# techpro-studio/NNToolkitCore

Hardware: AMD Instinct MI355X
Metric: audio frames/sec (whole node) (higher is better)
Workload: dtype f32

## Files before the change

include/nntoolkitcore_hip.h:

```cpp
#ifndef NNTOOLKITCORE_HIP_H
#define NNTOOLKITCORE_HIP_H

#include <stdbool.h>
#include <stddef.h>

#ifdef __cplusplus
extern "C" {
#endif


typedef struct { int mini_batch_size; } DefaultTrainingConfig;
typedef struct { int w; int b; int sum; } DefaultWeightsSize;
typedef struct { float *W; float *b; } DefaultWeights;

typedef void (*ActivationFunctionImpl)(void *, const float *, float *, int);
typedef void (*ActivationFunctionDerivative)(void *, const float *, const float *, float *, int);
typedef void (*ActivationImplementerDestroy)(void *);
typedef struct ActivationFunctionStruct *ActivationFunction;

ActivationFunction ActivationFunctionCreate(int size, ActivationImplementerDestroy destroy_fn, void *implementer,
                                            ActivationFunctionImpl function, ActivationFunctionDerivative derivative,
                                            ActivationFunctionDerivative cached_derivative);
void ActivationFunctionDestroy(ActivationFunction filter);
void ActivationFunctionApply(ActivationFunction filter, const float *input, float *output);
// ... 220 lines not shown
typedef struct {
    int nfft;
    int window_size;
    int noverlap;
    int step;
    int input_size;
    int nfreq;
    int ntime_series;
    float fft_normalization_factor;
} SpectrogramConfig;
typedef struct SpectrogramStruct *Spectrogram;

SpectrogramConfig SpectrogramConfigCreate(int nfft, int window_size, int noverlap, int input_size,
                                          float fft_normalization_factor);
Spectrogram SpectrogramCreatePSD(SpectrogramConfig config, int fs);
Spectrogram SpectrogramCreateMagnitude(SpectrogramConfig config);
SpectrogramConfig SpectrogramGetConfig(Spectrogram filter);
void SpectrogramSetWindowFunc(Spectrogram filter, window_fn fn);
void SpectrogramSetScaleFactor(Spectrogram filter, float factor);
void SpectrogramApply(Spectrogram filter, const float *input, float *output);
void SpectrogramDestroy(Spectrogram filter);

typedef struct {
    int n_mels;
    int n_fft;
    int sample_rate;
    float lower_hz;
    float upper_hz;
} MelFilterBankConfig;
typedef struct MelFilterBankStruct *MelFilterBank;
typedef struct LogMelSpectrogramStruct *LogMelSpectrogram;

MelFilterBankConfig MelFilterBankConfigCreate(int n_mels, int n_fft, int sample_rate, float lower_hz, float upper_hz);
MelFilterBank MelFilterBankCreate(MelFilterBankConfig config);
void MelFilterBankApply(MelFilterBank filter_bank, const float *spectrogram, float *mel_spectrogram, int timesteps);
void MelFilterBankDestroy(MelFilterBank filter_bank);
LogMelSpectrogram LogMelSpectrogramCreate(Spectrogram spectrogram, MelFilterBankConfig mel_filter_bank_config);
void LogMelSpectrogramApply(LogMelSpectrogram filter, const float *input, float *output);
void LogMelSpectrogramDestroy(LogMelSpectrogram filter);


int         nntk_hip_device_count(void);
int         nntk_hip_set_device(int device);
void        nntk_hip_set_stream(void *hip_stream);
void       *nntk_hip_get_stream(void);
int         nntk_hip_synchronize(void);
const char *nntk_last_error(void);
const char *nntk_version(void);
const char *nntk_build_source_hash(void);
int         nntk_hip_set_option(const char *name, const char *value);
int         nntk_hip_get_option(const char *name, int *value);
int         nntk_hip_device_status(void);
const char *nntk_hip_last_recurrent_kernel(void);
const char *nntk_hip_last_conv_kernel(void);
void        nntk_hip_profile_enable(int on);
int         nntk_hip_profile_get(const char *name, double *total_ms, long *launches, long *timesteps);

float *nntk_device_alloc(size_t n_floats);
void   nntk_device_free(float *ptr);
int    nntk_device_upload(float *dst_device, const float *src_host, size_t n_floats);
int    nntk_device_download(float *dst_host, const float *src_device, size_t n_floats);

int Conv1dSyncWeights(Conv1d filter);
int BatchNormSyncWeights(BatchNorm filter);
int GRUSyncWeights(GRU filter);
int LSTMSyncWeights(LSTM filter);
int RNNSyncWeights(RNN filter);
int DenseSyncWeights(Dense filter);
int TimeDistributedDenseSyncWeights(TimeDistributedDense filter);
int Conv1dLoadWeightsDevice(Conv1d filter, const float *d_block);
int BatchNormLoadWeightsDevice(BatchNorm filter, const float *d_block);
int GRULoadWeightsDevice(GRU filter, const float *d_block);
int LSTMLoadWeightsDevice(LSTM filter, const float *d_block);
int RNNLoadWeightsDevice(RNN filter, const float *d_block);
int DenseLoadWeightsDevice(Dense filter, const float *d_block);
int TimeDistributedDenseLoadWeightsDevice(TimeDistributedDense filter, const float *d_block);

#define NNTK_DIST_ID_BYTES 128
int  nntk_dist_get_unique_id(unsigned char id[NNTK_DIST_ID_BYTES]);
int  nntk_dist_init(const unsigned char id[NNTK_DIST_ID_BYTES], int rank, int world_size);
int  nntk_dist_rank(void);
int  nntk_dist_world_size(void);
int  nntk_dist_broadcast(float *host_block, size_t n_floats, int root);
int  nntk_dist_barrier(void);
int  nntk_dist_allreduce(float *host_block, size_t n_floats);
int  nntk_dist_allreduce_device(float *d_block, size_t n_floats);
int  nntk_dist_finalize(void);
void nntk_dist_shard_range(int n_utterances, int world_size, int rank, int *lo, int *hi);
int Conv1dBroadcastWeights(Conv1d filter, int root);
int BatchNormBroadcastWeights(BatchNorm filter, int root);
int GRUBroadcastWeights(GRU filter, int root);
int LSTMBroadcastWeights(LSTM filter, int root);
int RNNBroadcastWeights(RNN filter, int root);
int DenseBroadcastWeights(Dense filter, int root);
int TimeDistributedDenseBroadcastWeights(TimeDistributedDense filter, int root);

int Conv1dApplyInferenceBatch(Conv1d filter, const float *input, float *output, int batch);
int GRUApplyInferenceBatch(GRU filter, const float *input, float *output, int batch);
int LSTMApplyInferenceBatch(LSTM filter, const float *input, float *output, int batch);
int RNNApplyInferenceBatch(RNN filter, const float *input, float *output, int batch);
int TimeDistributedDenseApplyInferenceBatch(TimeDistributedDense filter, const float *input, float *output, int batch);
int SpectrogramApplyBatch(Spectrogram filter, const float *input, float *output, int batch);
int LogMelSpectrogramApplyBatch(LogMelSpectrogram filter, const float *input, float *output, int batch);

int SpectrogramApplyDevice(Spectrogram filter, const float *d_input ,
                           float *d_output , int batch);
// ... 267 lines not shown
```

nntoolkitcore_amd/capi.py:

```python
import ctypes as C
import os

_PKG = os.path.dirname(os.path.abspath(__file__))
LIB_PATH = os.path.join(_PKG, "lib", "libnntoolkitcore_hip.so")
if os.environ.get("NNTK_LIB"):
    LIB_PATH = os.path.abspath(os.environ["NNTK_LIB"])

fp = C.POINTER(C.c_float)
vp = C.c_void_p


class Conv1dConfig(C.Structure):
    _fields_ = [("input_feature_channels", C.c_int), ("output_feature_channels", C.c_int),
                ("kernel_size", C.c_int), ("stride", C.c_int), ("input_size", C.c_int), ("output_size", C.c_int)]


class ConvTrainingConfig(C.Structure):
    _fields_ = [("mini_batch_size", C.c_int)]


class DefaultGradient(C.Structure):
    _fields_ = [("d_W", fp), ("d_b", fp), ("d_X", fp)]


# ... 203 lines not shown
    "DenseGradientDestroy": (None, [C.POINTER(DefaultGradient)]),
    "DenseCalculateGradient": (None, [vp, C.POINTER(DefaultGradient), fp]),
    "ActivationFunctionCalculateGradient": (None, [vp, fp, fp, fp, fp]),
    "ActivationFunctionCalculateGradientDevice": (C.c_int, [vp, vp, vp, vp, vp, C.c_int]),
    "mean_squared_error": (C.c_float, [fp, fp, C.c_int, C.c_int]),
    "mean_squared_error_derivative": (None, [fp, fp, fp, C.c_int, C.c_int]),
    "categorical_crossentropy": (C.c_float, [fp, fp, C.c_int, C.c_int]),
    "categorical_crossentropy_derivative": (None, [fp, fp, fp, C.c_int, C.c_int]),
    "sgd_optimize": (C.c_int, [SGD, fp, fp, C.c_int]),
    "nntk_mean_squared_error_device": (C.c_int, [vp, vp, C.c_int, C.c_int, C.POINTER(C.c_float)]),
    "nntk_categorical_crossentropy_device": (C.c_int, [vp, vp, C.c_int, C.c_int, C.POINTER(C.c_float)]),
    "nntk_mean_squared_error_derivative_device": (C.c_int, [vp, vp, vp, C.c_int, C.c_int]),
    "nntk_categorical_crossentropy_derivative_device": (C.c_int, [vp, vp, vp, C.c_int, C.c_int]),
    "nntk_sgd_optimize_device": (C.c_int, [SGD, vp, vp, C.c_long]),
    "DenseDestroy": (None, [vp]),
    "TimeDistributedDenseConfigCreate": (TimeDistributedDenseConfig, [C.c_int, DenseConfig]),
    "TimeDistributedDenseCreateForInference": (vp, [TimeDistributedDenseConfig]),
    "TimeDistributedDenseGetWeights": (C.POINTER(DefaultWeights), [vp]),
    "TimeDistributedDenseApplyInference": (C.c_int, [vp, fp, fp]),
    "TimeDistributedDenseDestroy": (None, [vp]),
    "hamming_window": (None, [fp, C.c_int]),
    "hann_window": (None, [fp, C.c_int]),
    "ones": (None, [fp, C.c_int]),
    "periodic_hamming_window": (None, [fp, C.c_int]),
    "periodic_hann_window": (None, [fp, C.c_int]),
    "blackman_window": (None, [fp, C.c_int]),
    "SpectrogramConfigCreate": (SpectrogramConfig, [C.c_int, C.c_int, C.c_int, C.c_int, C.c_float]),
    "SpectrogramCreatePSD": (vp, [SpectrogramConfig, C.c_int]),
    "SpectrogramCreateMagnitude": (vp, [SpectrogramConfig]),
    "SpectrogramGetConfig": (SpectrogramConfig, [vp]),
    "SpectrogramSetWindowFunc": (None, [vp, vp]),
    "SpectrogramSetScaleFactor": (None, [vp, C.c_float]),
    "SpectrogramApply": (None, [vp, fp, fp]),
    "SpectrogramDestroy": (None, [vp]),
    "MelFilterBankConfigCreate": (MelFilterBankConfig, [C.c_int, C.c_int, C.c_int, C.c_float, C.c_float]),
    "MelFilterBankCreate": (vp, [MelFilterBankConfig]),
    "MelFilterBankApply": (None, [vp, fp, fp, C.c_int]),
    "MelFilterBankDestroy": (None, [vp]),
    "LogMelSpectrogramCreate": (vp, [vp, MelFilterBankConfig]),
    "LogMelSpectrogramApply": (None, [vp, fp, fp]),
    "LogMelSpectrogramDestroy": (None, [vp]),
    "nntk_hip_device_count": (C.c_int, []),
    "nntk_hip_set_device": (C.c_int, [C.c_int]),
    "nntk_hip_set_stream": (None, [vp]),
    "nntk_hip_get_stream": (vp, []),
    "nntk_hip_synchronize": (C.c_int, []),
    "nntk_last_error": (C.c_char_p, []),
    "nntk_version": (C.c_char_p, []),
    "nntk_build_source_hash": (C.c_char_p, []),
    "nntk_hip_set_option": (C.c_int, [C.c_char_p, C.c_char_p]),
    "nntk_hip_get_option": (C.c_int, [C.c_char_p, C.POINTER(C.c_int)]),
    "nntk_hip_device_status": (C.c_int, []),
    "nntk_hip_last_recurrent_kernel": (C.c_char_p, []),
    "nntk_hip_last_conv_kernel": (C.c_char_p, []),
    "nntk_hip_profile_enable": (None, [C.c_int]),
    "nntk_hip_profile_get": (C.c_int, [C.c_char_p, C.POINTER(C.c_double), C.POINTER(C.c_long), C.POINTER(C.c_long)]),
    "nntk_device_alloc": (vp, [C.c_size_t]),
    "nntk_device_free": (None, [vp]),
    "nntk_device_upload": (C.c_int, [vp, fp, C.c_size_t]),
    "nntk_device_download": (C.c_int, [fp, vp, C.c_size_t]),
    "nntk_dist_get_unique_id": (C.c_int, [C.c_char_p]),
    "nntk_dist_init": (C.c_int, [C.c_char_p, C.c_int, C.c_int]),
    "nntk_dist_rank": (C.c_int, []),
    "nntk_dist_world_size": (C.c_int, []),
    "nntk_dist_broadcast": (C.c_int, [fp, C.c_size_t, C.c_int]),
    "nntk_dist_barrier": (C.c_int, []),
    "nntk_dist_allreduce": (C.c_int, [fp, C.c_size_t]),
    "nntk_dist_allreduce_device": (C.c_int, [vp, C.c_size_t]),
    "nntk_dist_finalize": (C.c_int, []),
    "nntk_dist_shard_range": (None, [C.c_int, C.c_int, C.c_int, C.POINTER(C.c_int), C.POINTER(C.c_int)]),
    "Conv1dBroadcastWeights": (C.c_int, [vp, C.c_int]),
    "BatchNormBroadcastWeights": (C.c_int, [vp, C.c_int]),
    "GRUBroadcastWeights": (C.c_int, [vp, C.c_int]),
    "LSTMBroadcastWeights": (C.c_int, [vp, C.c_int]),
    "RNNBroadcastWeights": (C.c_int, [vp, C.c_int]),
    "DenseBroadcastWeights": (C.c_int, [vp, C.c_int]),
    "TimeDistributedDenseBroadcastWeights": (C.c_int, [vp, C.c_int]),
    "Conv1dSyncWeights": (C.c_int, [vp]),
    "BatchNormSyncWeights": (C.c_int, [vp]),
    "GRUSyncWeights": (C.c_int, [vp]),
    "LSTMSyncWeights": (C.c_int, [vp]),
    "RNNSyncWeights": (C.c_int, [vp]),
    "DenseSyncWeights": (C.c_int, [vp]),
    "TimeDistributedDenseSyncWeights": (C.c_int, [vp]),
    "Conv1dApplyInferenceBatch": (C.c_int, [vp, fp, fp, C.c_int]),
    "GRUApplyInferenceBatch": (C.c_int, [vp, fp, fp, C.c_int]),
    "LSTMApplyInferenceBatch": (C.c_int, [vp, fp, fp, C.c_int]),
    "RNNApplyInferenceBatch": (C.c_int, [vp, fp, fp, C.c_int]),
    "TimeDistributedDenseApplyInferenceBatch": (C.c_int, [vp, fp, fp, C.c_int]),
    "SpectrogramApplyBatch": (C.c_int, [vp, fp, fp, C.c_int]),
    "LogMelSpectrogramApplyBatch": (C.c_int, [vp, fp, fp, C.c_int]),
    "MelFilterBankApplyDevice": (C.c_int, [vp, vp, vp, C.c_int]),
    "LogMelSpectrogramApplyDevice": (C.c_int, [vp, vp, vp, C.c_int]),
    "SpectrogramApplyDevice": (C.c_int, [vp, vp, vp, C.c_int]),
    "Conv1dApplyDevice": (C.c_int, [vp, vp, vp, C.c_int]),
    "Conv1dBatchNormActivationApplyDevice": (C.c_int, [vp, vp, vp, vp, vp, C.c_int]),
    "Conv1dBatchNormActivationApplyDeviceFrag3": (C.c_int, [vp, vp, vp, vp, vp, C.c_int]),
    "BatchNormApplyDevice": (C.c_int, [vp, vp, vp, C.c_int]),
    "ActivationFunctionApplyDevice": (C.c_int, [vp, vp, vp, C.c_int]),
    "GRUApplyDevice": (C.c_int, [vp, vp, vp, C.c_int]),
    "GRUStack2ApplyDevice": (C.c_int, [vp, vp, vp, vp, C.c_int]),
    "GRUStack2ApplyInferenceBatch": (C.c_int, [vp, vp, fp, fp, C.c_int]),
    "LSTMApplyDevice": (C.c_int, [vp, vp, vp, C.c_int]),
    "nntk_frag3_floats": (C.c_size_t, [C.c_int, C.c_int, C.c_int]),
    "nntk_frag3_pack_device": (C.c_int, [vp, vp, C.c_int, C.c_int, C.c_int]),
    "nntk_frag3_unpack_device": (C.c_int, [vp, vp, C.c_int, C.c_int, C.c_int]),
# ... 194 lines not shown
```

nntoolkitcore_amd/csrc/hip/nntk_common.hpp:

```cpp
#pragma once
#include <hip/hip_runtime.h>
#include <math.h>
#include "nntk_shim.h"

hipStream_t nntk_stream();
int nntk_fail(const char *what, hipError_t err);
int nntk_fail_msg(const char *what);
enum { NNTK_SPAN_REC = 0, NNTK_SPAN_SPEC = 1 };
int nntk_prof_span_begin(int kind);
void nntk_prof_span_end(int idx, long launches, long units);

struct NntkOptions {
    int rec_persistent = -1;
    int rec_xw = -1;
    int rec_pingpong = -1;
    int rec_groups = 2;
    int rec_spin_us = 1000000;
    int rec_stream = -1;
    int rec_fused2 = -1;
    int rec_rr = -1;
    int rec_xf = -1;
    int rec_fk = -1;
    int rec_hf = -1;
    int rec_hf_pend = 1;
    int rec_bd = -1;
    int dense_frag3 = -1;
    int dense_f16x2 = -1;
    int train_outer_plain = -1;
    int train_bptt = -1;
    int spec_ppw = 0;
    int spec_variant = -1;
#ifdef NNTK_VARIANT_SPEC_DMA
    int spec_dma = -1;
#endif
    int bn_fast = 0;
    int gemm_tm_batch = -1;
    int conv_a4 = 1;
    int conv_flatk = -1;
    int conv_frag3_out = -1;
    int conv_store = -1;
    int gemm_split_bf16 = -1;
    int gemm_wide = -1;
    int conv_dbg = 0;
    int weights_check = -1;
};
const NntkOptions &nntk_options();

unsigned *nntk_fault_word();
int nntk_fault_enqueue_copy();
int nntk_persistent_disabled();
void nntk_persistent_launch_begin();
void nntk_persistent_launch_end();
bool nntk_weights_exact_only(const void *d_wp);
int nntk_cu_count();
void nntk_set_last_conv_kernel(const char *name);
void nntk_set_last_rec_kernel(const char *name);
int nntk_set_max_dynamic_lds(const void *kernel, size_t bytes);
int nntk_outer_mfma_launch(const float *d_A, const float *d_B, float *d_partial, long rows, int I, int K, int a_shift_T,
                           long rps, long seq_pitch, long row_pitch);
int nntk_resident_blocks(const void *kernel, int threads, size_t lds, int max_per_cu);

#define NNTK_STR_(x) #x
#define NNTK_STR(x) NNTK_STR_(x)

#define NNTK_HIP_TRY(expr)                                             \
    do {                                                               \
        hipError_t _e = (expr);                                        \
        if (_e != hipSuccess) return nntk_fail(#expr, _e);             \
    } while (0)

#define NNTK_LAUNCH_CHECK(name)                                        \
    do {                                                               \
        hipError_t _e = hipGetLastError();                             \
        if (_e != hipSuccess) return nntk_fail(name, _e);              \
    } while (0)

typedef float f32x4 __attribute__((ext_vector_type(4)));
typedef float f32x16 __attribute__((ext_vector_type(16)));

__device__ __forceinline__ float nntk_act(int kind, float x, float relu_a) {
    switch (kind) {
    case NNTK_ACT_SIGMOID: return 1.0f / (1.0f + expf(-x));
    case NNTK_ACT_TANH:    return tanhf(x);
    case NNTK_ACT_RELU: {
        float y = fmaxf(x, 0.0f);
        return relu_a != 1.0f ? y * relu_a : y;
    }
    case NNTK_ACT_LOG_EPS: return logf(x + relu_a);
    default: return x;
    }
}

__device__ __forceinline__ float nntk_fast_sigmoid(float x) {
    return __builtin_amdgcn_rcpf(1.0f + __builtin_amdgcn_exp2f(-1.44269504088896341f * x));
}
__device__ __forceinline__ float nntk_fast_tanh(float x) {
    const float e = __builtin_amdgcn_exp2f(-2.88539008177792681f * fabsf(x));
    const float r = (1.0f - e) * __builtin_amdgcn_rcpf(1.0f + e);
    return copysignf(r, x);
}
__device__ __forceinline__ float nntk_gate_act(int kind, float x, float a = 1.0f) {
    switch (kind) {
    case NNTK_ACT_SIGMOID: return nntk_fast_sigmoid(x);
    case NNTK_ACT_TANH:    return nntk_fast_tanh(x);
    case NNTK_ACT_RELU: {
        const float y = fmaxf(x, 0.0f);
        return a != 1.0f ? y * a : y;
    }
    default: return x;
// ... 5 lines not shown
```

nntoolkitcore_amd/csrc/hip/nntk_shim.h:

```cpp
#ifndef NNTK_SHIM_H
#define NNTK_SHIM_H

#include <stddef.h>

#ifdef __cplusplus
extern "C" {
#endif

enum {
    NNTK_ACT_NONE     = -1,
    NNTK_ACT_IDENTITY = 0,
    NNTK_ACT_SIGMOID  = 1,
    NNTK_ACT_TANH     = 2,
    NNTK_ACT_RELU     = 3,
    NNTK_ACT_SOFTMAX  = 4,
    NNTK_ACT_LOG_EPS  = 5,
    NNTK_ACT_CUSTOM   = 100
};

int         nntk_shim_device_count(void);
int         nntk_shim_set_device(int device);
int         nntk_shim_get_device(void);
void        nntk_shim_set_stream(void *stream);
void       *nntk_shim_get_stream(void);
int         nntk_shim_synchronize(void);
const char *nntk_shim_error(void);
void        nntk_shim_set_error(const char *msg);
void        nntk_shim_clear_error(void);

int nntk_shim_set_option(const char *name, const char *value);
int nntk_shim_get_option(const char *name, int *value);
int nntk_shim_take_fault(void);
int nntk_shim_persistent_disabled(void);
const char *nntk_shim_last_conv_kernel(void);
const char *nntk_shim_last_rec_kernel(void);
int nntk_shim_device_status(void);

void nntk_shim_profile_enable(int on);
int  nntk_shim_profile_get(const char *name, double *total_ms, long *launches, long *timesteps);

void *nntk_shim_malloc(size_t bytes);
void  nntk_shim_free(void *d_ptr);
void *nntk_shim_host_alloc(size_t bytes);
void  nntk_shim_host_free(void *ptr);
int   nntk_shim_upload(void *d_dst, const void *h_src, size_t bytes);
int   nntk_shim_upload_async(void *d_dst, const void *h_src, size_t bytes);
int   nntk_shim_download(void *h_dst, const void *d_src, size_t bytes);
int   nntk_shim_download_nocheck(void *h_dst, const void *d_src, size_t bytes);
int   nntk_shim_download_rows(void *h_dst, const void *d_src, size_t spitch, size_t width, size_t height);
int   nntk_shim_copy_d2d(void *d_dst, const void *d_src, size_t bytes);
int   nntk_shim_copy_rows_d2d(void *d_dst, const void *d_src, size_t spitch, size_t width, size_t height);
int   nntk_shim_memset(void *d_ptr, int value, size_t bytes);

void nntk_shim_conv_pack_sizes(int Cin, int Cout, int k, int *Cin_p, int *Cout_p);
int  nntk_shim_bn_derive(float *d_block, float eps, int C);
int  nntk_shim_split_bf16x3(const float *d_src, void *d_dst, int rows, int ktot);
void nntk_shim_weights_exact_only(const void *d_wp, int on);
int  nntk_shim_conv1d(const float *d_in, const float *d_wp, const float *d_bias, const float *d_bn,
                      float bn_eps, int act_kind, float relu_a, float *d_out,
                      int B, int T, int Cin, int Cout, int k, int stride, int Tout, int out_mode);

int  nntk_shim_conv1d_frag3(const float *d_in, const float *d_wp, const float *d_bias, const float *d_bn,
                            float bn_eps, int act_kind, float relu_a, float *d_out_f3,
                            int B, int T, int Cin, int Cout, int k, int stride, int Tout);
int nntk_shim_conv1d_flatk(const float *d_in, const float *d_wpf, const float *d_bias, const float *d_bn,
                           float bn_eps, int act_kind, float relu_a, float *d_out,
                           int B, int T, int Cin, int Cout, int k, int Tout);
size_t nntk_shim_conv1d_grad_scratch_floats(int Cin, int Cout, int k);
int nntk_shim_conv1d_grad(const float *d_in, const float *d_W, const float *d_dout, float *d_dW, float *d_db,
                          float *d_dX, float *d_scratch, int B, int T, int Cin, int Cout, int k, int stride, int Tout);

int nntk_shim_batch_norm(const float *d_in, const float *d_bn , float eps,
                         float *d_out, long rows, int C);
int nntk_shim_activation(int kind, float relu_a, int softmax_vector_size,
                         const float *d_in, float *d_out, long n_elems);

int nntk_shim_reverse_time(const float *d_in, float *d_out, long B, int T, int F);
int nntk_shim_reverse_time_varlen(const float *d_in, float *d_out, const int *d_len, long B, int T, int F);
int nntk_shim_upload_ints(int *d_dst, const int *h_src, long n);
int nntk_shim_stream_gather(const float *d_in, float *d_state, float *d_seq, const int *d_cnt, int B, int in_rows, int state_rows, int C);
int nntk_shim_spectrogram_rows(const float *d_in, const float *d_window, const float *d_twiddle, float *d_out,
                               int B, int row_stride, int nfft, int window_size, int step, int nfreq, int max_frames,
                               float fft_norm, int mode, float scale, const int *d_cnt,
                               const int *d_mel_tab, const float *d_mel_w, int n_mels, float eps, int do_log);
int nntk_shim_activation_grad(int kind, int vector_size, int vectors_per_call, const float *d_z, const float *d_a,
                              const float *d_dout, float *d_out, long n);
int nntk_shim_dense_grad(const float *d_x, const float *d_W , const float *d_dz, float *d_gW,
// ... 118 lines not shown
int nntk_shim_split2(const float *d_in, float *d_a, float *d_b, long rows, int C);
int nntk_shim_bd_merge(const float *d_of, const float *d_obr, float *d_out, const int *d_len, long B, int T, int H,
                       int return_sequences, int concat);
int nntk_shim_bd_scatter(const float *d_dout, float *d_of, float *d_ob, const int *d_len, long B, int T, int H,
                         int return_sequences, int concat, int reverse);
int nntk_shim_bd_accumulate(const float *d_dxf, const float *d_dxbr, float *d_dx, const int *d_len, long B, int T, int F);

int nntk_shim_rnn(const float *d_xw, const float *d_ut, const float *d_bh, const float *d_h0,
                  float *d_out, float *d_hT, float *d_work, int B, int T, int H,
                  int return_sequences, int act, float act_scale);
size_t nntk_shim_recurrent_work_floats(int B, int H);
int nntk_shim_rec_varlen(int G, const float *d_xw, const float *d_ut, const float *d_bh, const float *d_h0,
                         const float *d_c0, float *d_out, float *d_hT, float *d_cT, float *d_work, int B, int T, int H,
                         int return_sequences, const int *acts, const float *act_scales, const int *d_len, int T_max);
int nntk_shim_varlen_zero_pad(float *d_out, const int *d_len, int B, int T, int H);
int nntk_shim_gru(const float *d_xw, const float *d_ut, const float *d_bh,
                  const float *d_h0, float *d_out, float *d_hT, float *d_work,
                  int B, int T, int H, int return_sequences, const int acts[3], const float act_scales[3]);
int nntk_shim_lstm(const float *d_xw, const float *d_ut, const float *d_bh,
                   const float *d_h0, const float *d_c0, float *d_out, float *d_hT, float *d_cT,
                   float *d_work, int B, int T, int H, int return_sequences, const int acts[5], const float act_scales[5]);

size_t nntk_shim_lstm_rr_image_floats(int H, int in);
size_t nntk_shim_rr_image_floats_xf(int H, int in);
size_t nntk_shim_lstm_rr_work_floats(int B, int H);
size_t nntk_shim_rr_hseq_floats(int B, int T, int H);
int nntk_shim_lstm_rr_pack(const float *d_ut, const float *d_wp, float *d_img, int H, int in);
int nntk_shim_lstm_rr_pack_raw(const float *d_U , const float *d_W , float *d_img, int H, int in);
size_t nntk_shim_fk_image_floats(int H, int in);
int nntk_shim_fk_pack(const float *d_ut, const float *d_wp, float *d_img4, int H, int in);
int nntk_shim_fk_pack_raw(const float *d_U , const float *d_W , float *d_img4, int H, int in);
int nntk_shim_gru_rr(const float *d_x, const void *d_xf3, const float *d_img, const float *d_img4, const float *d_b4, const float *d_h0, float *d_out,
                     float *d_hseq, float *d_hT, float *d_work, int B, int T, int in, int H, int return_sequences, int x_tm, int out_tm);
int nntk_shim_gru_rr_train_forward(const float *d_x, const float *d_img, const float *d_b4, float *d_h, float *d_hU, float *d_Zg,
                                   float *d_hseq, float *d_work, int B, int T, int in, int H);
int nntk_shim_lstm_rr_train_forward(const float *d_x, const float *d_img, const float *d_bi, const float *d_bh,
                                    float *d_h, float *d_c, float *d_zifgo, float *d_hseq, float *d_work, int B, int T, int in, int H);
int nntk_shim_lstm_rr(const float *d_x, const void *d_xf3, const float *d_img, const float *d_img4, const float *d_bi, const float *d_bh,
                      const float *d_h0, const float *d_c0, float *d_out, float *d_out_h2 ,
                      float *d_hseq, float *d_hT, float *d_cT, float *d_work, int B, int T, int in, int H, int return_sequences);

int nntk_shim_rr_varlen(int cell, const float *d_x, const void *d_xf3, const float *d_img, const float *d_img4, const float *d_bi,
                        const float *d_bh, const float *d_h0, const float *d_c0, float *d_out, float *d_hseq, float *d_hT, float *d_cT,
                        float *d_work, const int *d_len, int B, int T, int in, int H, int return_sequences);

int nntk_shim_rr_bd(int cell, const void *d_xf3, const float *d_img, const float *d_img4, const float *d_bi, const float *d_bh,
                    const float *d_img_b, const float *d_img4_b, const float *d_bi_b, const float *d_bh_b, float *d_out, float *d_out_b,
                    int ldo, float *d_hseq, float *d_work, const int *d_len, int B, int T, int in, int H, int return_sequences);
int nntk_shim_rr_bd_fits(int T, int in, int ldo);

int nntk_shim_lstm_rr_hf_ok(int H, int in);
size_t nntk_shim_lstm_rr_hf_image_floats(int H, int in);
int nntk_shim_lstm_rr_pack_hf(const float *d_ut, const float *d_wp, float *d_img, int H, int in, float uscale, float wscale);
int nntk_shim_lstm_rr_hf(const void *d_xf3, const float *d_img, const float *d_bi, const float *d_bh, float *d_h2, float *d_work,
                         int B, int T, int in, int H, float z_scale);

size_t nntk_shim_frag3_floats(int B, int T, int C);
int nntk_shim_frag3_pack(const float *d_x, void *d_frag, int B, int T, int C);
int nntk_shim_frag3_pack_bd(const float *d_x, const int *d_len, void *d_frag, int B, int T, int C);
int nntk_shim_frag3_unpack(const void *d_frag, float *d_x, int B, int T, int C);
size_t nntk_shim_frag2h_floats(int B, int T, int C);
int nntk_shim_frag2h_pack(const float *d_x, void *d_frag, int B, int T, int C);
int nntk_shim_frag2h_unpack(const void *d_frag, float *d_x, int B, int T, int C);
int nntk_shim_split_f16x2(const float *d_src, void *d_dst, int rows, int ktot, float scale);
int nntk_shim_dense_frag2h(const void *d_frag, const void *d_wh2, float w_scale, const float *d_bias, int act_kind, float relu_a,
                           float *d_out, int B, int T, int K, int N, int probe);
int nntk_shim_dense_frag3(const void *d_frag, const float *d_wp, const float *d_bias, int act_kind, float relu_a,
                          float *d_out, int B, int T, int K, int N);

size_t nntk_shim_gru2_work_floats(int B, int H);
int nntk_shim_gru2(const float *d_xw1, const float *d_ut1, const float *d_bh1, const float *d_wt2,
                   const float *d_bi2, const float *d_ut2, const float *d_bh2, float *d_out, float *d_out1,
                   float *d_work, int B, int T, int H, int return_sequences);

int nntk_shim_rec_stream(int G, int is_lstm, const float *x, const float *d_wp, const float *d_bi,
                         const float *d_ut, const float *d_bh, float *d_h0, float *d_h1, float *d_c0, float *d_c1,
                         int cur, float *out, int T, int in, int H, int return_sequences,
                         const int *acts, const float *scales, unsigned *d_done, unsigned *flag, unsigned seq);

int nntk_shim_dist_unique_id(unsigned char *id128);
int nntk_shim_dist_init(const unsigned char *id128, int rank, int world);
int nntk_shim_dist_rank(void);
int nntk_shim_dist_world(void);
int nntk_shim_dist_broadcast_host(float *block, size_t n, int root);
int nntk_shim_add_into(float *d_dst, const float *d_src, long n);
int nntk_shim_dist_barrier(void);
int nntk_shim_dist_allreduce_device(float *d_block, size_t n);
int nntk_shim_dist_allreduce_host(float *block, size_t n);
int nntk_shim_dist_finalize(void);

int nntk_shim_spectrogram(const float *d_in, const float *d_window, const float *d_twiddle, float *d_out,
                          int B, int input_size, int nfft, int window_size, int step,
                          int nfreq, int nts, float fft_norm, int mode, float scale);

int nntk_shim_spectrogram_mel(const float *d_in, const float *d_window, const float *d_twiddle, float *d_out,
                              int B, int input_size, int nfft, int window_size, int step,
                              int nfreq, int nts, float fft_norm, int mode, float scale,
                              const int *d_mel_tab, const float *d_mel_w, int n_mels, float eps, int do_log);

#ifdef __cplusplus
}
#endif
#endif
```

nntoolkitcore_amd/csrc/hip/recurrent_fk.hip:

```cpp
#include "recurrent_rr_common.hpp"

typedef unsigned fk_v2u __attribute__((ext_vector_type(2)));
template <int LO, int HI, class F>
__device__ __forceinline__ void fk_for(F &&f) {
    if constexpr (LO < HI) {
        f(std::integral_constant<int, LO>{});
        fk_for<LO + 1, HI>(f);
    }
}
__host__ __device__ constexpr int fk_ring(int NKX, int NW) { return NW == 4 && NKX > 8 ? 2 : 4; }
#ifndef FK_ND_4
#define FK_ND_4 3
#endif
#ifndef FK_ND_4W
#define FK_ND_4W 4
#endif
#ifndef FK_LEAD_CAP
#define FK_LEAD_CAP 0
#endif
#ifndef FK_FIN_SLICED
#define FK_FIN_SLICED 0
#endif
#ifndef FK_FIN_VALU
#define FK_FIN_VALU 5
#endif
#ifndef FK_ND_2
#define FK_ND_2 8
#endif

#ifdef NNTK_REC_STAMPS
#ifndef FK_FINE_GS
#define FK_FINE_GS 2
#endif
#define FK_FINE(gs, k) do { if ((gs) == FK_FINE_GS) asm volatile("s_memtime %0" : "=s"(fine[k])); } while (0)
#define FK_FINE_OUT(gs, t) do { if ((gs) == FK_FINE_GS) { asm volatile("s_waitcnt lgkmcnt(0)" ::: "memory"); \
        if (p.stamp && blockIdx.x == 0 && w == 0 && lane == 0 && (t) >= 0) { for (int k_ = 0; k_ < 10; ++k_) p.stamp[(size_t)(t) * 64 + 48 + k_] = fine[k_]; } } } while (0)
#define FK_STAMP(t, i) do { if (p.stamp && blockIdx.x == 0 && w == 0 && lane == 0 && (t) >= 0) \
        p.stamp[(size_t)(t) * 64 + (i)] = __builtin_amdgcn_s_memtime(); } while (0)
#else
#define FK_STAMP(t, i) do {} while (0)
#define FK_FINE(gs, k) do {} while (0)
#define FK_FINE_OUT(gs, t) do {} while (0)
#endif

__host__ __device__ inline int fk_blocks_per_ct(int NKH, int NKX, int NW) { return NW * (NKH * 3 + NKX * 3); }
__host__ __device__ inline int fk_nmr(int NKH) { return NKH <= 16 ? 3 : 2; }
__host__ __device__ inline int fk_nmw(int NKX, int NW) { return NW == 4 && NKX > 8 ? 1 : 0; }
__host__ __device__ inline int fk_walk(int NGP, int NW, int ct, int ug, int pos) {
    const int g = pos / NW, j = pos % NW;
    return NW * ((g + ct) % NGP) + ((ug ^ j ^ (ct / NGP)) & (NW - 1));
}

template <bool RAW>
__global__ __launch_bounds__(256) void fk_pack_kernel(const float *__restrict__ ut, const float *__restrict__ wp,
                                                      rr_v4u *__restrict__ img, int H, int in, int Hj_p, int Hk_p, int Kin_p,
                                                      int NKH, int NKX, int NMR, int NW, int NCT) {
    const int NMW = fk_nmw(NKX, NW);
    const int n_ur = NW * NKH * NMR, n_wr = NW * NKX * NMW, n_ul = NW * NKH * (3 - NMR), bpc = fk_blocks_per_ct(NKH, NKX, NW);
    const long total = (long)NCT * bpc * 64;
    for (long e = blockIdx.x * (long)blockDim.x + threadIdx.x; e < total; e += (long)gridDim.x * blockDim.x) {
        const int l = (int)(e & 63);
        const long blk = e >> 6;
        const int ct = (int)(blk / bpc);
        int r = (int)(blk % bpc);
        int part, ug, pos, m;
        if (r < n_ur) { part = 0; m = r % NMR; pos = (r / NMR) % NKH; ug = r / (NMR * NKH); }
        else if (r < n_ur + n_wr) { r -= n_ur; part = 2; m = r % NMW; pos = (r / NMW) % NKX; ug = r / (NMW * NKX); }
        else if (r < n_ur + n_wr + n_ul) { r -= n_ur + n_wr; part = 0; const int nl = 3 - NMR; m = NMR + r % nl; pos = (r / nl) % NKH; ug = r / (nl * NKH); }
        else { r -= n_ur + n_wr + n_ul; part = 2; const int nl = 3 - NMW; m = NMW + r % nl; pos = (r / nl) % NKX; ug = r / (nl * NKX); }
        const int ks = fk_walk(part == 2 ? NKX / NW : NKH / NW, NW, ct, ug, pos);
        const int c = l & 31;
        const int g = c >> 3;
        const int j = 8 * (NW * ct + ug) + (c & 7);
        float v[8];
#pragma unroll
        for (int q = 0; q < 8; ++q) {
            const int k = 16 * ks + 8 * (l >> 5) + q;
            float val = 0.0f;
            if (j < H) {
                if (RAW) {
                    if (part == 2) { if (k < in) val = wp[(size_t)k * 4 * H + (size_t)g * H + j]; }
                    else if (k < H) val = ut[(size_t)k * 4 * H + (size_t)g * H + j];
                } else {
                    if (part == 2) { if (k < in) val = wp[((size_t)g * H + j) * Kin_p + k]; }
                    else if (k < H) val = ut[((size_t)g * Hj_p + j) * Hk_p + k];
                }
            }
            v[q] = val;
        }
        rr_v4u hi, mid, lo;
        rr_split8(v, hi, mid, lo);
        img[e] = m == 0 ? hi : m == 1 ? mid : lo;
    }
}

template <int NKH, int NKX, int CELL, int NW, int ND, bool VL = false, bool BD = false>
__device__ __forceinline__ void fk_body(const RRParams &p) {
    static_assert(!BD || VL, "BD: per-row lengths");
    constexpr int NMR = NKH <= 16 ? 3 : 2;
    constexpr int NMW = NW == 4 && NKX > 8 ? 1 : 0;
    constexpr int FK_RING = fk_ring(NKX, NW);
    constexpr bool BURST = FK_RING == 2;
    constexpr int NGH = NKH / NW, NGX = NKX / NW, NG = NGH + NGX;
    constexpr int NHF = 4 / NW;
    static_assert((NW == 2 || NW == 4) && NKH % NW == 0 && NKX % NW == 0 && NGX >= 1, "group schedule");
    static_assert((2 * NG) % ND == 0 && (2 * NG) % fk_ring(NKX, NW) == 0 && ND <= NGH, "staging / ring indices repeat every two steps at most");
    constexpr auto fk_lead = [](int q) constexpr {
        if (q >= NGH) return ND;
        if (!FK_LEAD_CAP) return ND;
        const int want = 2 + (q + 1) / 2, cap = NGX + q;
        const int l = want < cap ? want : cap;
        return l < ND ? l : ND;
    };
    constexpr int FIN_G = NW == 4 ? 1 : (NGX >= 4 ? 4 : NGX);
    extern __shared__ __attribute__((aligned(16))) char smem[];
    rr_v4u *ULs = reinterpret_cast<rr_v4u *>(smem);
    rr_v4u *WXs = ULs + NW * NKH * (3 - NMR) * 64;
    rr_v4u *ring = WXs + NW * NKX * (3 - NMW) * 64;
    unsigned *flg = reinterpret_cast<unsigned *>(ring + 4 * FK_RING * 3 * 64);
#define FK_FENCE() asm volatile("" ::: "memory")

    const int tid = threadIdx.x;
    const int lane = tid & 63;
    const int w = __builtin_amdgcn_readfirstlane(tid >> 6);
    const int hf = w / NW, ug = w % NW;
    const int n = lane & 31, kh = lane >> 5;
    const int bt = blockIdx.x % p.NBT;
    const int ct = blockIdx.x / p.NBT;
    const int ht_abs = p.b_base / 32 + bt * NHF + hf;
    const int b0 = p.b_base + bt * 32 * NHF;
    const int H = p.H;
    const int T = VL ? __builtin_amdgcn_readfirstlane(p.len[p.B + (b0 >> 6)]) : p.T;
    const int NKS = H >> 4;
    const bool bwd = BD && b0 >= p.bd_pad;
    const int rb0 = bwd ? b0 - p.bd_pad : b0;
    const int rows_valid = BD ? (p.bd_rows - rb0 < 32 * NHF ? (p.bd_rows > rb0 ? p.bd_rows - rb0 : 0) : 32 * NHF)
                              : p.B - b0 < 32 * NHF ? p.B - b0 : 32 * NHF;
    const int gi = NW * ct + ug;
    if (VL && T == 0) {
        if constexpr (BD) rr_bd_pass_state(p, b0, 32 * NHF, 8 * NW * ct, 8 * NW);
        else rr_vl_pass_state(p, b0, 32 * NHF, 8 * NW * ct, 8 * NW, CELL == 0);
        return;
    }
    const bool grp_ok = 8 * gi < H;

    const rr_v4u *img = (bwd ? p.img_b : p.img) + (size_t)ct * fk_blocks_per_ct(NKH, NKX, NW) * 64;
    rr_bf16x8 uh[NKH][NMR];
#pragma unroll
    for (int pos = 0; pos < NKH; ++pos)
#pragma unroll
        for (int m = 0; m < NMR; ++m) {
            uh[pos][m] = __builtin_bit_cast(rr_bf16x8, img[(((size_t)ug * NKH + pos) * NMR + m) * 64 + lane]);
            RR_PIN_A(uh[pos][m]);
        }
    rr_bf16x8 wr[NMW ? NKX : 1][NMW ? NMW : 1];
    if (NMW) {
#pragma unroll
        for (int pos = 0; pos < NKX; ++pos)
#pragma unroll
            for (int m = 0; m < NMW; ++m) {
                wr[pos][m] = __builtin_bit_cast(rr_bf16x8, img[(size_t)NW * NKH * NMR * 64 + (((size_t)ug * NKX + pos) * NMW + m) * 64 + lane]);
            }
    }
    {
        const rr_v4u *src = img + (size_t)(NW * NKH * NMR + NW * NKX * NMW) * 64;
        constexpr int n16 = (NW * NKH * (3 - NMR) + NW * NKX * (3 - NMW)) * 64;
        for (int e = tid; e < n16; e += 256) ULs[e] = src[e];
        for (int e = tid; e < 4 * FK_RING * 64; e += 256) flg[e] = 0u;
    }
    const int jf = 8 * gi + 4 * kh;
    float bsum[4][4];
    const float *const bi = bwd ? p.bi_b : p.bi, *const bh = bwd ? p.bh_b : p.bh;
#pragma unroll
    for (int g = 0; g < 4; ++g)
#pragma unroll
        for (int e = 0; e < 4; ++e)
            bsum[g][e] = jf + e < H ? bi[g * H + jf + e] + (bh ? bh[g * H + jf + e] : 0.0f) : 0.0f;
    float cst[4];
    {
        const int row = b0 + hf * 32 + n;
#pragma unroll
        for (int e = 0; e < 4; ++e) cst[e] = (p.c0 && row < p.B && jf + e < H) ? p.c0[(size_t)row * H + jf + e] : 0.0f;
    }
    int vlen = 0;
    float hkeep[VL && CELL == 0 ? 4 : 1];
    if constexpr (VL) {
        const int row = b0 + hf * 32 + n;
        vlen = row < p.B ? p.len[row] : 0;
        if constexpr (CELL == 0) {
#pragma unroll
            for (int e = 0; e < 4; ++e) hkeep[e] = (p.h0 && row < p.B && jf + e < H) ? p.h0[(size_t)row * H + jf + e] : 0.0f;
        }
    }
    const int hb_bytes = (int)p.hstep;
    auto rs_rd = [&](int t) __attribute__((always_inline)) {
        return __builtin_amdgcn_make_buffer_rsrc((void *)(t ? p.hseq + (size_t)(t - 1) * p.hstep : p.h0f), 0, t < T ? hb_bytes : 0, 0x00020000);
    };
    auto rs_wr = [&](int t) __attribute__((always_inline)) {
        return __builtin_amdgcn_make_buffer_rsrc((void *)(p.hseq + (size_t)t * p.hstep), 0, hb_bytes, 0x00020000);
    };
    auto rs_x = [&](int t) __attribute__((always_inline)) {
#ifdef FK_X_HOT
        return __builtin_amdgcn_make_buffer_rsrc((void *)(p.xf3), 0, t < T ? (int)p.xstep : 0, 0x00020000);
#endif
        return __builtin_amdgcn_make_buffer_rsrc((void *)(p.xf3 + (size_t)(t < T ? t : 0) * p.xstep), 0, t < T ? (int)p.xstep : 0, 0x00020000);
    };
    const int lane16 = lane * 16;
    const int ugh = (ug ^ (ct / NGH)) & (NW - 1), ugx = (ug ^ (ct / NGX)) & (NW - 1);
    const int hso = ht_abs * NKS * 3 * 1024;
    const int xso = ht_abs * p.NKSx * 3 * 1024;
    const int ldo = BD ? p.ldo : H;
    const long o_row_bytes = (long)(p.return_sequences ? p.T : 1) * ldo * 4;
    const long o_range = rows_valid * o_row_bytes;
    const __amdgpu_buffer_rsrc_t rso = __builtin_amdgcn_make_buffer_rsrc(
        (void *)((bwd ? p.out_b : p.out) + (size_t)rb0 * (o_row_bytes / 4)), 0, (int)(o_range < 0x7fffffffL ? o_range : 0x7fffffffL), 0x00020000);
    const bool row_ok = hf * 32 + n < rows_valid && grp_ok;
    const int out_vo = row_ok ? (int)((hf * 32 + n) * o_row_bytes) + jf * 4 : 0x7fff0000;
    const int pub_vo = grp_ok ? ((ht_abs * NKS + (gi >> 1)) * 3) * 1024 + (32 * (gi & 1) + n) * 16 + 8 * kh : RR_OOB_F;
    RR_BARRIER();

    using Tt = std::true_type;
    using Ff = std::false_type;
    using I0 = std::integral_constant<int, 0>;
    using I1 = std::integral_constant<int, 1>;
    rr_v4u S[ND][3];
    rr_v4u P[NW - 1][3];
    unsigned fl[NW - 1];
    rr_bf16x8 wa[2][3];
    rr_bf16x8 ulo[2];

    auto issue_own = [&](int g_h, int g_x, bool is_h, int si, int tq, int m0 = 0, int m1 = 3) __attribute__((always_inline)) {
        if (RR_DBG(1)) return;
        if (is_h) {
            const __amdgpu_buffer_rsrc_t rs = rs_rd(tq);
            const int ks = NW * ((g_h + ct) % NGH) + ugh;
            const int so = hso + ks * 3072;
            const int vo = lane16 + (ks < NKS ? 0 : RR_OOB_F);
#pragma unroll
            for (int m = 0; m < 3; ++m) {
                if (m < m0 || m >= m1) continue;
                S[si][m] = __builtin_amdgcn_raw_buffer_load_b128(rs, vo + m * 1024, so, 16 );
                RR_BOUND(tq ? 3 : 4, tq ? (size_t)(tq - 1) * p.hstep : 0, vo + m * 1024, so, tq < T ? hb_bytes : 0, 16);
            }
        } else {
            const __amdgpu_buffer_rsrc_t rs = rs_x(tq + 1);
            const int ks = NW * ((g_x + ct) % NGX) + ugx;
            const int so = xso + ks * 3072;
            const int vo = lane16 + (ks < p.NKSx ? 0 : RR_OOB_F);
#pragma unroll
            for (int m = 0; m < 3; ++m) {
                if (m < m0 || m >= m1) continue;
                S[si][m] = __builtin_amdgcn_raw_buffer_load_b128(rs, vo + m * 1024, so, 0);
                RR_BOUND(1, (size_t)(tq + 1) * p.xstep, vo + m * 1024, so, tq + 1 < T ? p.xstep : 0, 16);
            }
        }
    };
    auto probe = [&](int si) __attribute__((always_inline)) {
        unsigned mx = 0;
#pragma unroll
        for (int m = 0; m < 3; ++m) {
            const rr_v4u v = S[si][m];
            mx = max(mx, max(max(v.x, v.y), max(v.z, v.w)));
        }
        return __builtin_amdgcn_ballot_w64(mx == RR_PENDING);
    };
    const unsigned long long inject = p.spin_ticks == 0 ? ~0ull : 0ull;
    auto settle = [&](int g_h, int si, int tq) __attribute__((always_inline)) {
        {
            const unsigned long long t_start = __builtin_amdgcn_s_memrealtime();
            bool expired = p.spin_ticks == 0;
            while (!expired) {
                issue_own(g_h, 0, true, si, tq);
                if (probe(si) == 0) break;
                if (__hip_atomic_load(p.fault, __ATOMIC_RELAXED, __HIP_MEMORY_SCOPE_AGENT) != 0) { expired = true; break; }
                __builtin_amdgcn_s_sleep(1);
                expired = __builtin_amdgcn_s_memrealtime() - t_start > p.spin_ticks;
            }
            if (expired && lane == 0) __hip_atomic_fetch_or(p.fault, 1u, __ATOMIC_RELAXED, __HIP_MEMORY_SCOPE_AGENT);
        }
    };
    auto ring_put = [&](int si, int slot, unsigned seq, int piece) __attribute__((always_inline)) {
        rr_v4u *d = ring + ((w * FK_RING + slot) * 3) * 64 + lane;
        FK_FENCE();
#pragma unroll
        for (int m = 0; m < 3; ++m)
            if (piece < 0 || piece == m) d[m * 64] = S[si][m];
        FK_FENCE();
        if (piece < 0 || piece == 2) flg[(w * FK_RING + slot) * 64 + lane] = seq;
        FK_FENCE();
    };
    auto ring_word = [&](int j, int slot) __attribute__((always_inline)) {
        const int pw = hf * NW + (ug ^ j);
        FK_FENCE();
        fl[j - 1] = flg[(pw * FK_RING + slot) * 64 + lane];
        FK_FENCE();
    };
    auto ring_data = [&](int j, int slot, int m0, int m1) __attribute__((always_inline)) {
        const int pw = hf * NW + (ug ^ j);
        const rr_v4u *s = ring + ((pw * FK_RING + slot) * 3) * 64 + lane;
        FK_FENCE();
#pragma unroll
        for (int m = 0; m < 3; ++m)
            if (m >= m0 && m < m1) P[j - 1][m] = s[m * 64];
        FK_FENCE();
    };
    auto ring_check = [&](int slot, unsigned seq) __attribute__((always_inline)) {
        bool bad = false;
#pragma unroll
        for (int j = 1; j < NW; ++j) bad |= fl[j - 1] != seq;
        if (__builtin_amdgcn_ballot_w64(bad) != 0) {
            const unsigned long long t_start = __builtin_amdgcn_s_memrealtime();
            bool expired = false;
            while (!expired) {
                bad = false;
#pragma unroll
                for (int j = 1; j < NW; ++j) { ring_word(j, slot); bad |= fl[j - 1] != seq; }
                if (__builtin_amdgcn_ballot_w64(bad) == 0) break;
                if (__hip_atomic_load(p.fault, __ATOMIC_RELAXED, __HIP_MEMORY_SCOPE_AGENT) != 0) { expired = true; break; }
                __builtin_amdgcn_s_sleep(1);
                expired = __builtin_amdgcn_s_memrealtime() - t_start > p.spin_ticks;
            }
            if (expired && lane == 0) __hip_atomic_fetch_or(p.fault, 1u, __ATOMIC_RELAXED, __HIP_MEMORY_SCOPE_AGENT);
#pragma unroll
            for (int j = 1; j < (BURST ? NW : 2); ++j) ring_data(j, slot, 0, 3);
        }
    };
    float hn[4];
    rr_v4u olast = {0u, 0u, 0u, 0u};
    auto fin_unit = [&](int e, const f32x16 &acc, int t) __attribute__((always_inline)) {
        if (RR_DBG(2)) return;
        float zc[4];
#pragma unroll
        for (int g = 0; g < 4; ++g) zc[g] = acc[4 * g + e] + bsum[g][e];
        if (RR_DBG(64)) { hn[e] = zc[0] + zc[1] + zc[2] + zc[3] + cst[e]; return; }
        if (CELL == 1) {
            const float zg = nntk_fast_sigmoid(zc[0]);
            const float rg = nntk_fast_sigmoid(zc[1]);
            const float ht = nntk_fast_tanh(fmaf(rg, zc[2], zc[3]));
            hn[e] = fmaf(-zg + 1.0f, ht, zg * cst[e]);
            if constexpr (VL) hn[e] = t < vlen ? hn[e] : cst[e];
            cst[e] = hn[e];
        } else {
            const float ig = nntk_fast_sigmoid(zc[0]);
            const float fg = nntk_fast_sigmoid(zc[1]);
            const float gg = nntk_fast_tanh(zc[2]);
            const float og = nntk_fast_sigmoid(zc[3]);
            const float cn = fmaf(fg, cst[e], ig * gg);
            if constexpr (VL) {
                const bool live = t < vlen;
                hn[e] = live ? og * nntk_fast_tanh(cn) : hkeep[e];
                cst[e] = live ? cn : cst[e];
                hkeep[e] = hn[e];
            } else {
            cst[e] = cn;
            hn[e] = og * nntk_fast_tanh(cn);
            }
        }
    };
    auto fin_store = [&](int t) __attribute__((always_inline)) {
        if (RR_DBG(2)) return;
        if (!RR_DBG(128)) {
            unsigned sh0, sm0, sl0, sh1, sm1, sl1;
            rr_split_pair(hn[0], hn[1], sh0, sm0, sl0);
            rr_split_pair(hn[2], hn[3], sh1, sm1, sl1);
            const fk_v2u a = {(unsigned)min(sh0, 0xfffffffeu), (unsigned)min(sh1, 0xfffffffeu)};
            const fk_v2u b = {(unsigned)min(sm0, 0xfffffffeu), (unsigned)min(sm1, 0xfffffffeu)};
            const fk_v2u c = {(unsigned)min(sl0, 0xfffffffeu), (unsigned)min(sl1, 0xfffffffeu)};
            const __amdgpu_buffer_rsrc_t rs = rs_wr(t);
            __builtin_amdgcn_raw_buffer_store_b64(a, rs, pub_vo, 0, RR_ST_AUX );
            __builtin_amdgcn_raw_buffer_store_b64(b, rs, pub_vo + 1024, 0, RR_ST_AUX);
            __builtin_amdgcn_raw_buffer_store_b64(c, rs, pub_vo + 2048, 0, RR_ST_AUX);
            RR_BOUND(3, (size_t)t * p.hstep, pub_vo + 2048, 0, hb_bytes, 8);
        }
        olast = (rr_v4u){__float_as_uint(hn[0]), __float_as_uint(hn[1]), __float_as_uint(hn[2]), __float_as_uint(hn[3])};
        if (!RR_DBG(1024)) {
            int vo = (row_ok && p.return_sequences && p.out) ? out_vo + t * H * 4 : 0x7fff0000;
            if constexpr (BD)
                vo = (row_ok && p.return_sequences && t < vlen) ? out_vo + (bwd ? vlen - 1 - t : t) * ldo * 4 : 0x7fff0000;
            __builtin_amdgcn_raw_buffer_store_b128(olast, rso, vo, 0, 0);
            RR_BOUND(2, (size_t)b0 * o_row_bytes, vo, 0, o_range < 0x7fffffffL ? o_range : 0x7fffffffL, 16);
        }
    };

    auto mark_next = [&](int t) __attribute__((always_inline)) {
        if (RR_DBG(128)) return;
        const __amdgpu_buffer_rsrc_t rs2 = rs_wr(t + 1 < T ? t + 1 : t);
        const int vo2 = t + 1 < T ? pub_vo : RR_OOB_F;
        const fk_v2u pend = {RR_PENDING, RR_PENDING};
        __builtin_amdgcn_raw_buffer_store_b64(pend, rs2, vo2, 0, RR_ST_AUX);
        __builtin_amdgcn_raw_buffer_store_b64(pend, rs2, vo2 + 1024, 0, RR_ST_AUX);
        __builtin_amdgcn_raw_buffer_store_b64(pend, rs2, vo2 + 2048, 0, RR_ST_AUX);
        RR_BOUND(3, (size_t)(t + 1 < T ? t + 1 : t) * p.hstep, vo2 + 2048, 0, hb_bytes, 8);
    };

    constexpr int PA[6] = {0, 2, 1, 0, 1, 0}, PB[6] = {2, 0, 1, 1, 0, 0};
    auto lds_fetch_a = [&](bool is_h, int pos, int buf) __attribute__((always_inline)) {
        if (is_h) {
            if (NMR == 2) ulo[buf] = __builtin_bit_cast(rr_bf16x8, ULs[(ug * NKH + pos) * 64 + lane]);
        } else {
#pragma unroll
            for (int m = NMW; m < 3; ++m) wa[buf][m] = __builtin_bit_cast(rr_bf16x8, WXs[((ug * NKX + pos) * (3 - NMW) + (m - NMW)) * 64 + lane]);
        }
    };
    auto mult = [&](f32x16 &acc, bool is_h, int pos, int buf, const rr_v4u (&bsrc)[3], int j0, int j1) __attribute__((always_inline)) {
        if (RR_DBG(16)) return;
        rr_bf16x8 b[3];
#pragma unroll
        for (int m = 0; m < 3; ++m) b[m] = __builtin_bit_cast(rr_bf16x8, bsrc[m]);
#pragma unroll
        for (int pr = 0; pr < 6; ++pr) {
            if (pr < j0 || pr >= j1) continue;
            rr_bf16x8 av;
            if (is_h) av = (NMR == 2 && PA[pr] == 2) ? ulo[buf] : uh[pos][PA[pr] < NMR ? PA[pr] : 0];
            else av = PA[pr] < NMW ? wr[NMW ? pos : 0][NMW ? PA[pr] : 0] : wa[buf][PA[pr]];
            acc = __builtin_amdgcn_mfma_f32_32x32x16_bf16(av, b[PB[pr]], acc, 0, 0, 0);
        }
    };

    auto issue_sched = [&](int gs, int par, int t, int k, int m0, int m1) __attribute__((always_inline)) {
        int seen = 0;
#pragma unroll
        for (int L = 1; L <= ND; ++L) {
            const int r = gs + L, q = r % NG;
            if (fk_lead(q) != L) continue;
            if (seen++ != k) continue;
            const bool qh = q < NGH;
            issue_own(qh ? q : 0, qh ? 0 : q - NGH, qh, (par * NG + r) % ND, t + r / NG, m0, m1);
        }
    };
    auto step = [&](auto par_tag, auto hp_tag, int t, f32x16 &acc, f32x16 &accn) __attribute__((always_inline)) {
        constexpr int PAR = decltype(par_tag)::value;
        constexpr bool HP = decltype(hp_tag)::value;
        fk_for<(HP ? 0 : NGH), NG>([&](auto gs_tag) __attribute__((always_inline)) {
            constexpr int gs = decltype(gs_tag)::value;
            const bool is_h = gs < NGH;
            const int pos0 = NW * (is_h ? gs : gs - NGH);
            const int gidx = PAR * NG + gs;
            const int si = gidx % ND, slot = gidx % FK_RING;
            const int si1 = (gidx + 1) % ND, slot1 = (gidx + 1) % FK_RING;
            const unsigned seq = (unsigned)((t + 1) * NG + gs) + 1u;
            const int q1 = (gs + 1) % NG, t1 = t + (gs + 1 >= NG ? 1 : 0);
            const bool h1 = q1 < NGH;
            f32x16 &a = is_h ? acc : accn;
            FK_STAMP(t, gs);
            if (gs == NGH) {
#pragma unroll
                for (int r = 0; r < 16; ++r) accn[r] = 0.0f;
            }
#define FK_PIN() __builtin_amdgcn_sched_barrier(0)
            const bool LATE = FK_LEAD_CAP && gs == NG - 1;
            const bool chk1 = h1 && !LATE && !RR_DBG(4) && !RR_DBG(1);
            unsigned mx0 = 0, mx1 = 0, mx2 = 0;
#ifdef NNTK_REC_STAMPS
            unsigned long long fine[10] = {0, 0, 0, 0, 0, 0, 0, 0, 0, 0};
#endif
            FK_FINE(gs, 0);
            mult(a, is_h, pos0, 0, S[si], 0, 1); FK_PIN();
#pragma unroll
            for (int j = 1; j < NW; ++j) ring_word(j, slot);
            if (chk1) { const rr_v4u v = S[si1][0]; mx0 = max(max(v.x, v.y), max(v.z, v.w)); asm volatile("" : "+v"(mx0)); }
            FK_PIN();
            mult(a, is_h, pos0, 0, S[si], 1, 2); FK_PIN();
            ring_data(1, slot, 0, 3);
            if (BURST && NW == 4) ring_data(2, slot, 0, 3);
            if (chk1) { const rr_v4u v = S[si1][1]; mx1 = max(mx0, max(max(v.x, v.y), max(v.z, v.w))); asm volatile("" : "+v"(mx1)); }
            FK_PIN();
            mult(a, is_h, pos0, 0, S[si], 2, 3); FK_PIN();
            if (BURST && NW == 4) ring_data(3, slot, 0, 3);
            if (chk1) { const rr_v4u v = S[si1][2]; mx2 = max(mx1, max(max(v.x, v.y), max(v.z, v.w))); asm volatile("" : "+v"(mx2)); }
            lds_fetch_a(is_h, pos0 + 1, 1); FK_PIN();
            FK_FINE(gs, 1);
            {
                bool bad = false;
                if (!RR_DBG(512)) {
#pragma unroll
                    for (int j = 1; j < NW; ++j) bad |= fl[j - 1] != seq;
                }
                unsigned long long pend = chk1 ? __builtin_amdgcn_ballot_w64(mx2 == RR_PENDING) | inject : 0ull;
                if (t1 <= 0) pend = 0ull;
                if (__builtin_expect((pend | __builtin_amdgcn_ballot_w64(bad)) != 0, 0)) {
                    if (pend != 0) settle(q1, si1, t1);
                    if (!RR_DBG(512)) ring_check(slot, seq);
                }
            }
            FK_FINE(gs, 2);
#ifdef FK_COARSE_GS
            if (gs == FK_COARSE_GS) FK_STAMP(t, 40);
#endif
            if (!RR_DBG(512) && !LATE) ring_put(si1, slot1, seq + 1u, 0);
            FK_PIN();
            mult(a, is_h, pos0, 0, S[si], 3, 4); FK_PIN();
            if (!RR_DBG(512) && !LATE) ring_put(si1, slot1, seq + 1u, 1);
            FK_PIN();
            mult(a, is_h, pos0, 0, S[si], 4, 5); FK_PIN();
            if (!RR_DBG(512) && !LATE) ring_put(si1, slot1, seq + 1u, 2);
            FK_PIN();
            mult(a, is_h, pos0, 0, S[si], 5, 6); FK_PIN();
            if (HP && gs == 0) { mark_next(t); FK_PIN(); }
#ifdef FK_COARSE_GS
            if (gs == FK_COARSE_GS) FK_STAMP(t, 41);
#endif
            FK_FINE(gs, 3);
            const int gx = gs - NGH;
            const bool fin_here = FK_FIN_SLICED && HP && !is_h && gx < FIN_G;
#pragma unroll
            for (int j = 1; j < NW; ++j) {
                mult(a, is_h, pos0 + j, j & 1, P[j - 1], 0, 2); if (!fin_here) FK_PIN();
                if (j + 1 < NW && !BURST) ring_data(j + 1, slot, 0, 1);
                issue_sched(gs, PAR, t, j - 1, 0, 1); if (!fin_here) FK_PIN();
                if (j + 1 < NW) lds_fetch_a(is_h, pos0 + j + 1, (j + 1) & 1);
                else lds_fetch_a(h1, NW * (h1 ? q1 : q1 - NGH), 0);
                if (!fin_here) FK_PIN();
                mult(a, is_h, pos0 + j, j & 1, P[j - 1], 2, 4); if (!fin_here) FK_PIN();
                if (j + 1 < NW && !BURST) ring_data(j + 1, slot, 1, 2);
                issue_sched(gs, PAR, t, j - 1, 1, 2); if (!fin_here) FK_PIN();
                mult(a, is_h, pos0 + j, j & 1, P[j - 1], 4, 6); if (!fin_here) FK_PIN();
                if (j + 1 < NW && !BURST) ring_data(j + 1, slot, 2, 3);
                issue_sched(gs, PAR, t, j - 1, 2, 3); if (!fin_here) FK_PIN();
                FK_FINE(gs, 3 + j);
#ifdef FK_COARSE_GS
                if (gs == FK_COARSE_GS) FK_STAMP(t, 41 + j);
#endif
            }
#pragma unroll
            for (int k = NW - 1; k < 3; ++k) issue_sched(gs, PAR, t, k, 0, 3);
            if (fin_here) {
#pragma unroll
                for (int e = 0; e < 4; ++e)
                    if (e * FIN_G / 4 == gx) fin_unit(e, acc, t);
                if (gx == FIN_G - 1) fin_store(t);
#pragma unroll
                for (int k = 0; k < 6 * (NW - 1); ++k) {
                    __builtin_amdgcn_sched_group_barrier(0x008, 1, 0);
                    __builtin_amdgcn_sched_group_barrier(0x002, FK_FIN_VALU, 0);
                    if (k % 2 == 1) __builtin_amdgcn_sched_group_barrier(0x030, 1, 0);
                    else __builtin_amdgcn_sched_group_barrier(0x100, 1, 0);
                }
            }
            if (LATE) {
                if (h1 && t1 > 0 && !RR_DBG(4) && !RR_DBG(1)) {
                    const unsigned long long pend = probe(si1) | inject;
                    if (__builtin_expect(pend != 0, 0)) settle(q1, si1, t1);
                }
                if (!RR_DBG(512)) ring_put(si1, slot1, seq + 1u, -1);
            }
            __builtin_amdgcn_sched_barrier(0);
            FK_FINE_OUT(gs, t);
            if (!FK_FIN_SLICED && HP && gs == NGH - 1) {
#pragma unroll
                for (int e = 0; e < 4; ++e) fin_unit(e, acc, t);
                fin_store(t);
                FK_STAMP(t, 33);
                __builtin_amdgcn_sched_barrier(0);
            }
            if (FK_FIN_SLICED && HP && !is_h && gx == FIN_G - 1) FK_STAMP(t, 33);
        });
    };

    f32x16 accA, accB;
#pragma unroll
    for (int r = 0; r < 16; ++r) { accA[r] = 0.0f; accB[r] = 0.0f; }
    {
#pragma unroll
        for (int r = NGH; r < NGH + ND; ++r) {
            const int q = r % NG;
            if (r - fk_lead(q) >= NGH) continue;
            const bool qh = q < NGH;
            issue_own(qh ? q : 0, qh ? 0 : q - NGH, qh, (NG + r) % ND, -1 + r / NG);
        }
        ring_put((NG + NGH) % ND, (NG + NGH) % FK_RING, (unsigned)NGH + 1u, -1);
        lds_fetch_a(false, 0, 0);
    }
    step(I1{}, Ff{}, -1, accB, accA);
    for (int t = 0; t < T; t += 2) {
        step(I0{}, Tt{}, t, accA, accB);
        if (t + 1 >= T) break;
        step(I1{}, Tt{}, t + 1, accB, accA);
    }
    if constexpr (BD) {
        int b0e = rb0;
        asm volatile("" : "+s"(b0e));
        const int row = b0e + hf * 32 + n;
        if (row < p.bd_rows && grp_ok && !p.return_sequences)
            *reinterpret_cast<rr_v4u *>((bwd ? p.out_b : p.out) + (size_t)row * ldo + jf) = olast;
    } else {
        int b0e = b0;
        asm volatile("" : "+s"(b0e));
        const int row = b0e + hf * 32 + n;
        if (row < p.B && grp_ok) {
            if (!p.return_sequences && p.out) *reinterpret_cast<rr_v4u *>(p.out + (size_t)row * H + jf) = olast;
            if (p.hT) *reinterpret_cast<rr_v4u *>(p.hT + (size_t)row * H + jf) = olast;
            if (p.cT) *reinterpret_cast<rr_v4u *>(p.cT + (size_t)row * H + jf) =
                (rr_v4u){__float_as_uint(cst[0]), __float_as_uint(cst[1]), __float_as_uint(cst[2]), __float_as_uint(cst[3])};
        }
    }
}
template <int NKH, int NKX, int NW, int ND, bool VL = false, bool BD = false>
__global__ __launch_bounds__(256) void lstm_fk_kernel(RRParams p) { fk_body<NKH, NKX, 0, NW, ND, VL, BD>(p); }
template <int NKH, int NKX, int NW, int ND, bool VL = false, bool BD = false>
__global__ __launch_bounds__(256) void gru_fk_kernel(RRParams p) { fk_body<NKH, NKX, 1, NW, ND, VL, BD>(p); }

static bool fk_shape(int H, int in, int *NKH, int *NKX, int *NW) {
    if ((H % 16) != 0 || H <= 128 || H > 256 || in <= 64 || in > 256) return false;
    const int on = nntk_options().rec_fk;
    if (on == 0 || (on < 0 && in <= 128)) return false;
    *NKH = 16;
    *NKX = in <= 128 ? 8 : 16;
    *NW = 4;
#ifdef FK_NW2_WIDE
    if (in > 128) *NW = 2;
#endif
    return true;
}
static size_t fk_lds_bytes(int NKH, int NKX, int NW) {
    return (size_t)(NW * NKH * (3 - fk_nmr(NKH)) + NW * NKX * (3 - fk_nmw(NKX, NW)) + 4 * fk_ring(NKX, NW) * 3) * 1024 + 4 * fk_ring(NKX, NW) * 64 * 4;
}
extern "C" size_t nntk_shim_fk_image_floats(int H, int in) {
    int NKH, NKX, NW;
    if (!fk_shape(H, in, &NKH, &NKX, &NW)) return 0;
    return (size_t)((H + 8 * NW - 1) / (8 * NW)) * fk_blocks_per_ct(NKH, NKX, NW) * 256;
}
static int fk_pack(bool raw, const float *d_u, const float *d_w, float *d_img, int H, int in) {
    int NKH, NKX, NW;
    if (!fk_shape(H, in, &NKH, &NKX, &NW)) return nntk_fail_msg("fk_pack: shape not taken by the full-K register-resident kernel");
    const int Hj_p = (H + 15) & ~15, Hk_p = (H + 31) & ~31;
    int Kin_p, N_p;
    nntk_shim_conv_pack_sizes(in, 4 * H, 1, &Kin_p, &N_p);
    const int NCT = (H + 8 * NW - 1) / (8 * NW), NMR = NKH <= 16 ? 3 : 2;
    const long total = (long)NCT * fk_blocks_per_ct(NKH, NKX, NW) * 64;
    long g = (total + 255) / 256;
    if (g > 4096) g = 4096;
    if (raw) hipLaunchKernelGGL(fk_pack_kernel<true>, dim3((unsigned)g), dim3(256), 0, nntk_stream(), d_u, d_w, (rr_v4u *)d_img, H, in, 0, 0, 0, NKH, NKX, NMR, NW, NCT);
    else     hipLaunchKernelGGL(fk_pack_kernel<false>, dim3((unsigned)g), dim3(256), 0, nntk_stream(), d_u, d_w, (rr_v4u *)d_img, H, in, Hj_p, Hk_p, Kin_p, NKH, NKX, NMR, NW, NCT);
    NNTK_LAUNCH_CHECK("fk_pack_kernel");
    return 0;
}
extern "C" int nntk_shim_fk_pack(const float *d_ut, const float *d_wp, float *d_img, int H, int in) { return fk_pack(false, d_ut, d_wp, d_img, H, in); }
extern "C" int nntk_shim_fk_pack_raw(const float *d_U, const float *d_W, float *d_img, int H, int in) { return fk_pack(true, d_U, d_W, d_img, H, in); }

int nntk_fk_launch(RRParams q, const float *d_imgfk, const float *d_imgfk_b, int cell, size_t *launches) {
    int NKH, NKX, NW;
    if (!d_imgfk || !q.xf3 || q.x_tm || q.out_tm || !fk_shape(q.H, q.in, &NKH, &NKX, &NW)) return 1;
    const bool bd = q.out_b != nullptr;
    if (bd && (!d_imgfk_b || !q.len)) return 1;
    void (*kern)(RRParams) = nullptr;
    if (bd) {
        if (cell == 1) kern = NKX == 8 ? gru_fk_kernel<16, 8, 4, FK_ND_4, true, true> : gru_fk_kernel<16, 16, 4, FK_ND_4W, true, true>;
        else kern = NKX == 8 ? lstm_fk_kernel<16, 8, 4, FK_ND_4, true, true> : lstm_fk_kernel<16, 16, 4, FK_ND_4W, true, true>;
    } else if (q.len) {
        if (cell == 1) kern = NKX == 8 ? gru_fk_kernel<16, 8, 4, FK_ND_4, true> : gru_fk_kernel<16, 16, 4, FK_ND_4W, true>;
        else kern = NKX == 8 ? lstm_fk_kernel<16, 8, 4, FK_ND_4, true> : lstm_fk_kernel<16, 16, 4, FK_ND_4W, true>;
    } else if (cell == 1) kern = NKX == 8 ? gru_fk_kernel<16, 8, 4, FK_ND_4> : gru_fk_kernel<16, 16, 4, FK_ND_4W>;
    else kern = NKX == 8 ? lstm_fk_kernel<16, 8, 4, FK_ND_4> : lstm_fk_kernel<16, 16, 4, FK_ND_4W>;
#ifdef FK_NW2_WIDE
    if (NW == 2 && (q.len || bd)) return 1;
    if (NW == 2) kern = cell == 1 ? gru_fk_kernel<16, 16, 2, FK_ND_2> : lstm_fk_kernel<16, 16, 2, FK_ND_2>;
#endif
    const size_t lds = fk_lds_bytes(NKH, NKX, NW);
    if (lds > 160 * 1024) return 1;
    if (nntk_set_max_dynamic_lds((const void *)kern, lds)) return -1;
    const int NCT = (q.H + 8 * NW - 1) / (8 * NW);
    const int rows = 128 / NW;
    const int resident = nntk_resident_blocks((const void *)kern, 256, lds, 1);
    const int tiles_per_launch = resident / NCT;
    if (tiles_per_launch < 1) return 1;
    q.img = (const rr_v4u *)d_imgfk;
    if (bd) q.img_b = (const rr_v4u *)d_imgfk_b;
    q.NCT = NCT;
    const int nbt_total = (q.B + rows - 1) / rows;
    for (int bt0 = 0; bt0 < nbt_total; bt0 += tiles_per_launch) {
        const int nbt = nbt_total - bt0 < tiles_per_launch ? nbt_total - bt0 : tiles_per_launch;
        q.NBT = nbt; q.b_base = bt0 * rows;
        hipLaunchKernelGGL(kern, dim3((unsigned)(nbt * NCT)), dim3(256), lds, nntk_stream(), q);
    }
    if (launches) *launches = (size_t)((nbt_total + tiles_per_launch - 1) / tiles_per_launch);
    static const char *const names[2][3] = {{"lstm_fk_kernel<16,8,4>", "lstm_fk_kernel<16,16,4>", "lstm_fk_kernel<16,16,2>"}, {"gru_fk_kernel<16,8,4>", "gru_fk_kernel<16,16,4>", "gru_fk_kernel<16,16,2>"}};
    static const char *const bd_names[2][2] = {{"lstm_fk_kernel<16,8,4,bd>", "lstm_fk_kernel<16,16,4,bd>"}, {"gru_fk_kernel<16,8,4,bd>", "gru_fk_kernel<16,16,4,bd>"}};
    nntk_set_last_rec_kernel(bd ? bd_names[cell == 1][NKX == 16] : names[cell == 1][NW == 2 ? 2 : NKX == 16]);
    return 0;
}
```

nntoolkitcore_amd/csrc/hip/recurrent_rr.hip:

```cpp
#include "recurrent_rr_common.hpp"

__host__ __device__ inline int rr_blocks_per_ct(int KH, int KX) { return 4 * KH * 2 * 2 + 4 * KH * 2 + 4 * KX * 2 * 3; }

template <bool RAW>
__global__ __launch_bounds__(256) void rr_pack_kernel(const float *__restrict__ ut, const float *__restrict__ wp,
                                                      rr_v4u *__restrict__ img, int H, int in, int Hj_p, int Hk_p, int Kin_p,
                                                      int KH, int KX, int NCT, float uscale = 0.0f, float wscale = 1.0f) {
    const int bpc = rr_blocks_per_ct(KH, KX);
    const long total = (long)NCT * bpc * 64;
    for (long e = blockIdx.x * (long)blockDim.x + threadIdx.x; e < total; e += (long)gridDim.x * blockDim.x) {
        const int l = (int)(e & 63);
        const long blk = e >> 6;
        const int ct = (int)(blk / bpc);
        int r = (int)(blk % bpc);
        int part, w, i, mt, m;
        const int n_uh = 4 * KH * 4, n_ul = 4 * KH * 2;
        if (r < n_uh) { part = 0; m = r & 1; mt = (r >> 1) & 1; i = (r >> 2) % KH; w = (r >> 2) / KH; }
        else if (r < n_uh + n_ul) { r -= n_uh; part = 1; m = 2; mt = r & 1; i = (r >> 1) % KH; w = (r >> 1) / KH; }
        else { r -= n_uh + n_ul; part = 2; m = r % 3; mt = (r / 3) & 1; i = (r / 6) % KX; w = (r / 6) / KX; }
        const int c = 32 * mt + (l & 31);
        const int g = (c >> 3) & 3;
        const int j = 16 * ct + 8 * ((c >> 2) & 1) + 4 * (c >> 5) + (c & 3);
        const int ks = part == 2 ? w * KX + i : w * KH + i;
        float v[8];
// ... 743 lines not shown
    *KH = 8;
    *KX = in <= 64 ? 1 : in <= 128 ? 2 : in <= 256 ? 4 : 0;
    return *KX != 0;
}
static size_t rr_lds_bytes(int KH, int KX, bool train = false, bool hf = false) {
    const bool ulr = hf || KX > 2 || (RR_ULR8 && KH == 8 && !train);
    return (size_t)((ulr ? 0 : 4 * KH * 2) + 4 * KX * 6 + 32) * 1024 + 32 * RR_HX_LD * 4 + 3 * 32 * RR_HS_LD * 4;
}
static size_t rr_step_bytes(int B, int H) { return (size_t)((B + 63) / 64) * 2 * (H / 16) * 3 * 1024; }

extern "C" size_t nntk_shim_lstm_rr_image_floats(int H, int in) {
    int KH, KX;
    if (!rr_shape(H, in, false, &KH, &KX)) return 0;
    return (size_t)((H + 15) / 16) * rr_blocks_per_ct(KH, KX) * 256;
}
extern "C" size_t nntk_shim_rr_image_floats_xf(int H, int in) {
    int KH, KX;
    if (!rr_shape(H, in, true, &KH, &KX)) return 0;
    return (size_t)((H + 15) / 16) * rr_blocks_per_ct(KH, KX) * 256;
}
extern "C" size_t nntk_shim_lstm_rr_work_floats(int B, int H) {
    const size_t nht = (size_t)(B + 127) / 128 * 4;
    return rr_step_bytes(B, H) / 4 + nht * RR_FLAGS;
}
extern "C" size_t nntk_shim_rr_hseq_floats(int B, int T, int H) { return (size_t)T * (rr_step_bytes(B, H) / 4); }
extern "C" int nntk_shim_lstm_rr_pack(const float *d_ut, const float *d_wp, float *d_img, int H, int in) {
    int KH, KX;
    if (!rr_shape(H, in, true, &KH, &KX)) return nntk_fail_msg("lstm_rr_pack: shape not taken by the register-resident kernel");
    const int Hj_p = (H + 15) & ~15, Hk_p = (H + 31) & ~31;
    int Kin_p, N_p;
    nntk_shim_conv_pack_sizes(in, 4 * H, 1, &Kin_p, &N_p);
    const int NCT = (H + 15) / 16;
    const long total = (long)NCT * rr_blocks_per_ct(KH, KX) * 64;
    long g = (total + 255) / 256;
    if (g > 4096) g = 4096;
    hipLaunchKernelGGL(rr_pack_kernel<false>, dim3((unsigned)g), dim3(256), 0, nntk_stream(), d_ut, d_wp, (rr_v4u *)d_img, H, in,
                       Hj_p, Hk_p, Kin_p, KH, KX, NCT);
    NNTK_LAUNCH_CHECK("rr_pack_kernel");
    return 0;
}
extern "C" int nntk_shim_lstm_rr_pack_raw(const float *d_U, const float *d_W, float *d_img, int H, int in) {
    int KH, KX;
    if (!rr_shape(H, in, true, &KH, &KX)) return nntk_fail_msg("lstm_rr_pack_raw: shape not taken by the register-resident kernel");
    const int NCT = (H + 15) / 16;
    const long total = (long)NCT * rr_blocks_per_ct(KH, KX) * 64;
    long g = (total + 255) / 256;
    if (g > 4096) g = 4096;
    hipLaunchKernelGGL(rr_pack_kernel<true>, dim3((unsigned)g), dim3(256), 0, nntk_stream(), d_U, d_W, (rr_v4u *)d_img, H, in,
                       0, 0, 0, KH, KX, NCT);
    NNTK_LAUNCH_CHECK("rr_pack_kernel");
    return 0;
}

int nntk_fk_launch(RRParams q, const float *d_imgfk, const float *d_imgfk_b, int cell, size_t *launches);
struct RRIo {
    const float *img4;
    const float *x; const void *xf3; float *out; float *hseq; float *work;
    const float *h0, *c0; float *hT, *cT; float *c_cache, *z_cache;
    int x_tm, out_tm;
    float *out_h2;
    int hf;
    float z_scale;
    const int *len;
    const float *img_b, *img4_b, *bi_b, *bh_b;
    float *out_b;
    int bd_rows, ldo;
};
static int rr_launch(const RRIo &io, const float *d_img, const float *d_bi, const float *d_bh,
                     int B, int T, int in, int H, int return_sequences, int cell);

extern "C" int nntk_shim_lstm_rr(const float *d_x, const void *d_xf3, const float *d_img, const float *d_img4, const float *d_bi, const float *d_bh,
                                 const float *d_h0, const float *d_c0, float *d_out, float *d_out_h2, float *d_hseq, float *d_hT, float *d_cT,
                                 float *d_work, int B, int T, int in, int H, int return_sequences) {
    RRIo io = {d_img4, d_x, d_xf3, d_out, d_hseq, d_work, d_h0, d_c0, d_hT, d_cT, nullptr, nullptr, 0, 0, d_out_h2, 0, 0.0f, nullptr};
    return rr_launch(io, d_img, d_bi, d_bh, B, T, in, H, return_sequences, 0);
}
extern "C" int nntk_shim_rr_varlen(int cell, const float *d_x, const void *d_xf3, const float *d_img, const float *d_img4, const float *d_bi,
                                   const float *d_bh, const float *d_h0, const float *d_c0, float *d_out, float *d_hseq, float *d_hT, float *d_cT,
                                   float *d_work, const int *d_len, int B, int T, int in, int H, int return_sequences) {
    if (!d_len) return nntk_fail_msg("rr_varlen: no lengths");
    RRIo io = {d_img4, d_x, d_xf3, d_out, d_hseq, d_work, d_h0, cell == 1 ? d_h0 : d_c0, d_hT, cell == 1 ? nullptr : d_cT, nullptr, nullptr, 0, 0,
               nullptr, 0, 0.0f, d_len};
    return rr_launch(io, d_img, d_bi, d_bh, B, T, in, H, return_sequences, cell);
}
static bool rr_tile_fits(int T, int in, int ow) { return (double)64 * T * in * 4 < 2.0e9 && (double)64 * T * ow * 4 < 2.0e9; }
extern "C" int nntk_shim_rr_bd_fits(int T, int in, int ldo) { return rr_tile_fits(T, in, ldo); }
extern "C" int nntk_shim_rr_bd(int cell, const void *d_xf3, const float *d_img, const float *d_img4, const float *d_bi, const float *d_bh,
                               const float *d_img_b, const float *d_img4_b, const float *d_bi_b, const float *d_bh_b, float *d_out, float *d_out_b,
                               int ldo, float *d_hseq, float *d_work, const int *d_len, int B, int T, int in, int H, int return_sequences) {
    if (!d_len || !d_xf3 || !d_out || !d_out_b) return nntk_fail_msg("rr_bd: no lengths / input / output");
    if (B <= 0 || T <= 0) return 0;
    if (!d_img4 || !d_img4_b) d_img4 = d_img4_b = nullptr;
    RRIo io = {d_img4, nullptr, d_xf3, d_out, d_hseq, d_work, nullptr, nullptr, nullptr, nullptr, nullptr, nullptr, 0, 0, nullptr, 0, 0.0f, d_len,
               d_img_b, d_img4_b, d_bi_b, d_bh_b, d_out_b, B, ldo};
    return rr_launch(io, d_img, d_bi, d_bh, 2 * ((B + 63) / 64) * 64, T, in, H, return_sequences, cell);
}
extern "C" int nntk_shim_lstm_rr_hf_ok(int H, int in) {
    int KH, KX;
    return rr_shape_hf(H, in, &KH, &KX) && nntk_options().rec_hf != 0;
}
extern "C" size_t nntk_shim_lstm_rr_hf_image_floats(int H, int in) {
    int KH, KX;
    if (!rr_shape_hf(H, in, &KH, &KX)) return 0;
    return (size_t)((H + 15) / 16) * rr_blocks_per_ct(KH, KX) * 256;
}
extern "C" int nntk_shim_lstm_rr_pack_hf(const float *d_ut, const float *d_wp, float *d_img, int H, int in, float uscale, float wscale) {
    int KH, KX;
    if (!rr_shape_hf(H, in, &KH, &KX)) return nntk_fail_msg("lstm_rr_pack_hf: shape not taken");
    const int Hj_p = (H + 15) & ~15, Hk_p = (H + 31) & ~31;
    int Kin_p, N_p;
    nntk_shim_conv_pack_sizes(in, 4 * H, 1, &Kin_p, &N_p);
    const int NCT = (H + 15) / 16;
    const long total = (long)NCT * rr_blocks_per_ct(KH, KX) * 64;
    long g = (total + 255) / 256;
    if (g > 4096) g = 4096;
    hipLaunchKernelGGL(rr_pack_kernel<false>, dim3((unsigned)g), dim3(256), 0, nntk_stream(), d_ut, d_wp, (rr_v4u *)d_img, H, in,
                       Hj_p, Hk_p, Kin_p, KH, KX, NCT, uscale, wscale);
    NNTK_LAUNCH_CHECK("rr_pack_kernel");
    return 0;
}
extern "C" int nntk_shim_lstm_rr_hf(const void *d_xf3, const float *d_img, const float *d_bi, const float *d_bh, float *d_h2, float *d_work,
                                    int B, int T, int in, int H, float z_scale) {
    RRIo io = {nullptr, nullptr, d_xf3, nullptr, d_h2, d_work, nullptr, nullptr, nullptr, nullptr, nullptr, nullptr, 0, 0, nullptr, 1, z_scale, nullptr};
    return rr_launch(io, d_img, d_bi, d_bh, B, T, in, H, 1, 0);
}
extern "C" int nntk_shim_gru_rr(const float *d_x, const void *d_xf3, const float *d_img, const float *d_img4, const float *d_b4, const float *d_h0, float *d_out,
                                float *d_hseq, float *d_hT, float *d_work, int B, int T, int in, int H, int return_sequences, int x_tm, int out_tm) {
    RRIo io = {d_img4, d_x, d_xf3, d_out, d_hseq, d_work, d_h0, d_h0, d_hT, nullptr, nullptr, nullptr, x_tm, out_tm, nullptr, 0, 0.0f};
    return rr_launch(io, d_img, d_b4, nullptr, B, T, in, H, return_sequences, 1);
}
extern "C" int nntk_shim_gru_rr_train_forward(const float *d_x, const float *d_img, const float *d_b4, float *d_h, float *d_hU, float *d_Zg,
                                              float *d_hseq, float *d_work, int B, int T, int in, int H) {
    RRIo io = {nullptr, d_x, nullptr, d_h, d_hseq, d_work, nullptr, nullptr, nullptr, nullptr, d_hU, d_Zg, 0, 0, nullptr, 0, 0.0f};
    return rr_launch(io, d_img, d_b4, nullptr, B, T, in, H, 1, 1);
}
extern "C" int nntk_shim_lstm_rr_train_forward(const float *d_x, const float *d_img, const float *d_bi, const float *d_bh,
                                               float *d_h, float *d_c, float *d_zifgo, float *d_hseq, float *d_work, int B, int T, int in, int H) {
    RRIo io = {nullptr, d_x, nullptr, d_h, d_hseq, d_work, nullptr, nullptr, nullptr, nullptr, d_c, d_zifgo, 0, 0, nullptr, 0, 0.0f};
    return rr_launch(io, d_img, d_bi, d_bh, B, T, in, H, 1, 0);
}

extern "C" int nntk_shim_rr_train_forward_vl(int cell, const float *d_x, const float *d_img, const float *d_bi, const float *d_bh,
                                             const float *d_h0, const float *d_c0, float *d_h, float *d_c, float *d_z, float *d_hT, float *d_cT,
                                             float *d_hseq, float *d_work, const int *d_len, int B, int T, int in, int H) {
    if (!d_len) return nntk_fail_msg("rr_train_forward_vl: no lengths");
    RRIo io = {nullptr, d_x, nullptr, d_h, d_hseq, d_work, d_h0, cell == 1 ? d_h0 : d_c0, d_hT, cell == 1 ? nullptr : d_cT, d_c, d_z, 0, 0,
               nullptr, 0, 0.0f, d_len};
    return rr_launch(io, d_img, d_bi, d_bh, B, T, in, H, 1, cell);
}

template <int KH, int KX>
static void (*rr_pick(int cell, bool train, bool xf, bool vl = false, bool bd = false))(RRParams) {
    if (bd) return cell == 1 ? gru_rr_kernel<KH, KX, false, true, true, true> : lstm_rr_kernel<KH, KX, false, true, false, true, true>;
    if (vl && train) {
        if constexpr (KH == 4 && KX == 1) return cell == 1 ? nullptr : lstm_rr_kernel<KH, KX, true, false, false, true>;
        else return cell == 1 ? gru_rr_kernel<KH, KX, true, false, true> : lstm_rr_kernel<KH, KX, true, false, false, true>;
    }
    if (vl) {
        if (cell == 1) return xf ? gru_rr_kernel<KH, KX, false, true, true> : gru_rr_kernel<KH, KX, false, false, true>;
        return xf ? lstm_rr_kernel<KH, KX, false, true, false, true> : lstm_rr_kernel<KH, KX, false, false, false, true>;
    }
    if (cell == 1) return train ? gru_rr_kernel<KH, KX, true, false> : xf ? gru_rr_kernel<KH, KX, false, true> : gru_rr_kernel<KH, KX, false, false>;
    return train ? lstm_rr_kernel<KH, KX, true, false> : xf ? lstm_rr_kernel<KH, KX, false, true> : lstm_rr_kernel<KH, KX, false, false>;
}

static int rr_launch(const RRIo &io, const float *d_img, const float *d_bi, const float *d_bh,
                     int B, int T, int in, int H, int return_sequences, int cell) {
    if (B <= 0 || T <= 0) return 0;
    const bool xf = io.xf3 != nullptr;
    const bool train = io.c_cache != nullptr;
    if (xf && (train || io.x_tm)) return 1;
    const bool vl = io.len != nullptr;
    if (vl && (io.x_tm || io.out_tm || io.hf || io.out_h2)) return nntk_fail_msg("lstm_rr: lengths with a stacked / frag2h call");
    const bool bd = io.out_b != nullptr;
    if (bd && (!vl || !xf || io.h0 || io.hT || io.cT)) return nntk_fail_msg("lstm_rr: a bidirectional call needs lengths, a frag3 x and no carried state");
    if (!xf && !io.x) return nntk_fail_msg("lstm_rr: no input");
    if (!io.hseq || !io.work) return nntk_fail_msg("lstm_rr: no hand-off buffer");
    if (io.x_tm && (double)T * B * in * 4 >= 2.0e9) return 1;
    if (io.out_tm && (!return_sequences || !io.out || (double)T * B * H * 4 >= 2.0e9)) return 1;
    if (io.out_h2 && (io.out || io.img4 || train || !return_sequences)) return nntk_fail_msg("lstm_rr: frag2h output with an f32 output / on the full-K family");
    const NntkOptions &opt = nntk_options();
    if (opt.rec_rr == 0 || opt.rec_persistent == 0 || nntk_persistent_disabled()) return 1;
    int KH, KX;
    const bool hf = io.hf != 0;
    if (!(hf ? rr_shape_hf(H, in, &KH, &KX) : rr_shape(H, in, xf, &KH, &KX))) return 1;
    if (!xf && ((((size_t)io.x) & 15) != 0 || (in % 4) != 0)) return 1;
    if (hf && (KH != 8 || cell != 0 || !xf || train || io.h0 || io.out || io.out_h2 || io.img4 || !return_sequences || opt.rec_hf == 0)) return 1;
    const int NCT = H / 16;
    if (!rr_tile_fits(T, in, bd ? io.ldo : H)) return 1;
    void (*kern)(RRParams) = nullptr;
    if (KH == 8 && KX == 2) kern = rr_pick<8, 2>(cell, train, xf, vl, bd);
    else if (KH == 8 && KX == 1) kern = rr_pick<8, 1>(cell, train, xf, vl, bd);
    else if (KH == 4 && KX == 4) kern = rr_pick<4, 4>(cell, train, xf, vl, bd);
    else if (KH == 4 && KX == 2) kern = rr_pick<4, 2>(cell, train, xf, vl, bd);
    else if (KH == 4 && KX == 1) kern = rr_pick<4, 1>(cell, train, xf, vl, bd);
    const bool hfp = hf && opt.rec_hf_pend != 0 && KX != 4;
    if (hf) kern = KX == 4 ? lstm_rr_kernel<8, 4, false, true, true> : KX == 2 ? lstm_rr_kernel<8, 2, false, true, true> : lstm_rr_kernel<8, 1, false, true, true>;
    if (hfp) kern = KX == 2 ? lstm_rr_hfp_kernel<8, 2> : lstm_rr_hfp_kernel<8, 1>;
    if (!kern) return 1;
    const size_t lds = rr_lds_bytes(KH, KX, train, hf);
    if (lds > 160 * 1024) return 1;
    if (nntk_set_max_dynamic_lds((const void *)kern, lds)) return -1;
    const int resident = nntk_resident_blocks((const void *)kern, 256, lds, 1);
    const int tiles_per_launch = resident / NCT;
    if (tiles_per_launch < 1) return 1;
    unsigned *fault = nntk_fault_word();
    if (!fault) return 1;
    const size_t step = hf ? rr_step_bytes(B, H) / 3 * 2 : rr_step_bytes(B, H);
    if (step >= (size_t)RR_OOB_F) return 1;
    const int nbt_total = (B + 63) / 64;
    const size_t xstep = (size_t)nbt_total * 2 * ((in + 15) / 16) * 3 * 1024;
    if (xf && xstep >= (size_t)RR_OOB_F) return 1;
    unsigned *flags = reinterpret_cast<unsigned *>(io.work + step / 4);
    if (nntk_shim_memset(io.work, 0, step + (size_t)((B + 127) / 128) * 4 * RR_FLAGS * sizeof(unsigned))) return -1;
    if (nntk_shim_memset(io.hseq, 0xff, step * (size_t)(T < 2 ? T : 2))) return -1;
    if (io.h0) {
        long g = ((long)nbt_total * 2 * NCT * 64 + 255) / 256;
        if (g > 2048) g = 2048;
        hipLaunchKernelGGL(rr_tile_h0_kernel, dim3((unsigned)g), dim3(256), 0, nntk_stream(), io.h0, (rr_v4u *)io.work, B, H, H / 16);
    }
    RRParams q;
    q.x = io.x; q.img = (const rr_v4u *)d_img; q.bi = d_bi; q.bh = d_bh;
    q.h0f = (char *)io.work; q.hseq = (char *)io.hseq; q.hstep = step;
    q.xf3 = (const char *)io.xf3; q.xstep = xstep; q.NKSx = (in + 15) / 16;
    q.c0 = io.c0; q.cT = io.cT; q.hT = io.hT; q.out = io.out;
    q.c_cache = io.c_cache; q.z_cache = io.z_cache;
    q.x_tm = io.x_tm; q.out_tm = io.out_tm;
    q.fault = fault;
    q.spin_ticks = (unsigned long long)(opt.rec_spin_us > 0 ? opt.rec_spin_us : 0) * 100ull;
    q.B = B; q.T = T; q.H = H; q.in = in; q.NCT = NCT; q.return_sequences = return_sequences;
    q.NHT = nbt_total * 2;
    q.out_h2 = (char *)io.out_h2; q.h2step = rr_step_bytes(B, H) / 3 * 2;
    q.z_scale = io.z_scale;
    q.len = io.len; q.h0 = io.h0;
    q.img_b = (const rr_v4u *)io.img_b; q.bi_b = io.bi_b; q.bh_b = io.bh_b; q.out_b = io.out_b;
    q.bd_pad = bd ? B / 2 : 0; q.bd_rows = io.bd_rows; q.ldo = io.ldo;
#ifdef NNTK_REC_STAMPS
    q.stamp = nullptr;
    const char *stamp_path = getenv("NNTK_REC_STAMP_FILE");
    if (stamp_path) {
        if (hipMalloc((void **)&q.stamp, (size_t)(T + 1) * 64 * 8) != hipSuccess) return nntk_fail_msg("stamp alloc");
        (void)hipMemset(q.stamp, 0, (size_t)(T + 1) * 64 * 8);
    }
#endif
#ifdef NNTK_RR_BOUNDS
    static unsigned long long *g_bounds = nullptr;
    if (!g_bounds) {
        if (hipMalloc((void **)&g_bounds, 64) != hipSuccess) return nntk_fail_msg("bounds alloc");
        (void)hipMemset(g_bounds, 0, 64);
    }
    q.bounds = g_bounds;
    g_rr_bounds = g_bounds;
#endif
    const int span = nntk_prof_span_begin(NNTK_SPAN_REC);
    nntk_persistent_launch_begin();
    size_t launches = (size_t)(nbt_total + tiles_per_launch - 1) / tiles_per_launch;
    int took4 = 1;
    if (xf && !train && io.img4 && !io.out_tm) {
        q.flags = flags;
        took4 = nntk_fk_launch(q, io.img4, io.img4_b, cell, &launches);
        if (took4 < 0) { nntk_persistent_launch_end(); return -1; }
    }
    if (took4 == 1)
    for (int bt0 = 0; bt0 < nbt_total; bt0 += tiles_per_launch) {
        const int nbt = nbt_total - bt0 < tiles_per_launch ? nbt_total - bt0 : tiles_per_launch;
        q.NBT = nbt; q.b_base = bt0 * 64;
        q.flags = flags + (size_t)bt0 * 2 * RR_FLAGS;
        hipLaunchKernelGGL(kern, dim3((unsigned)(nbt * NCT)), dim3(256), lds, nntk_stream(), q);
    }
    const int copy_rc = nntk_fault_enqueue_copy();
    nntk_persistent_launch_end();
    if (copy_rc) return -1;
    nntk_prof_span_end(span, (long)launches, T);
#ifdef NNTK_REC_STAMPS
    if (q.stamp) {
        (void)hipStreamSynchronize(nntk_stream());
        unsigned long long *hs = (unsigned long long *)malloc((size_t)(T + 1) * 64 * 8);
        (void)hipMemcpy(hs, q.stamp, (size_t)(T + 1) * 64 * 8, hipMemcpyDeviceToHost);
        FILE *f = fopen(stamp_path, "wb");
        if (f) { fwrite(hs, 8, (size_t)(T + 1) * 64, f); fclose(f); }
        free(hs); (void)hipFree(q.stamp);
    }
#endif
    NNTK_LAUNCH_CHECK("lstm_rr_kernel");
    static const char *const names[2][2][3] = {{{"lstm_rr_kernel<4,1>", "lstm_rr_kernel<4,2>", "lstm_rr_kernel<4,4>"}, {"lstm_rr_kernel<8,1>", "lstm_rr_kernel<8,2>", ""}},
                                               {{"gru_rr_kernel<4,1>", "gru_rr_kernel<4,2>", "gru_rr_kernel<4,4>"}, {"gru_rr_kernel<8,1>", "gru_rr_kernel<8,2>", ""}}};
    static const char *const bd_names[2][2][3] = {{{"lstm_rr_kernel<4,1,bd>", "lstm_rr_kernel<4,2,bd>", "lstm_rr_kernel<4,4,bd>"}, {"lstm_rr_kernel<8,1,bd>", "lstm_rr_kernel<8,2,bd>", ""}},
                                                  {{"gru_rr_kernel<4,1,bd>", "gru_rr_kernel<4,2,bd>", "gru_rr_kernel<4,4,bd>"}, {"gru_rr_kernel<8,1,bd>", "gru_rr_kernel<8,2,bd>", ""}}};
    if (bd && took4 == 1) nntk_set_last_rec_kernel(bd_names[cell == 1][KH == 8][KX == 1 ? 0 : KX == 2 ? 1 : 2]);
    else if (hf && !hfp && KX != 4) nntk_set_last_rec_kernel(KX == 2 ? "lstm_rr_kernel<8,2,flags,hf>" : "lstm_rr_kernel<8,1,flags,hf>");
    else if (hf) nntk_set_last_rec_kernel(KX == 4 ? "lstm_rr_kernel<8,4,hf>" : KX == 2 ? "lstm_rr_kernel<8,2,hf>" : "lstm_rr_kernel<8,1,hf>");
    else if (took4 == 1) nntk_set_last_rec_kernel(names[cell == 1][KH == 8][KX == 1 ? 0 : KX == 2 ? 1 : 2]);
    return 0;
}
```

nntoolkitcore_amd/csrc/hip/runtime.hip:

```cpp
#include "nntk_common.hpp"
#include <stdio.h>
#include <string.h>
#include <vector>

#include <atomic>
#include <mutex>
#include <stdlib.h>

static thread_local hipStream_t t_stream = nullptr;
static thread_local char g_err[512] = "";

hipStream_t nntk_stream() { return t_stream; }

int nntk_fail(const char *what, hipError_t err) {
    snprintf(g_err, sizeof(g_err), "HIP error in %s: %s", what, hipGetErrorString(err));
    return -1;
}
int nntk_fail_msg(const char *what) {
    snprintf(g_err, sizeof(g_err), "%s", what);
    return -1;
}

static NntkOptions g_opt;
static std::once_flag g_opt_once;
static std::mutex g_opt_mutex;

struct OptDesc { const char *name; const char *env; int NntkOptions::*field; };
static const OptDesc g_opt_table[] = {
    {"rec_persistent", "NNTK_REC_PERSISTENT", &NntkOptions::rec_persistent},
    {"rec_xw", "NNTK_REC_XW", &NntkOptions::rec_xw},
    {"rec_pingpong", "NNTK_REC_PINGPONG", &NntkOptions::rec_pingpong},
    {"rec_groups", "NNTK_REC_GROUPS", &NntkOptions::rec_groups},
    {"rec_spin_us", "NNTK_REC_SPIN_US", &NntkOptions::rec_spin_us},
    {"rec_stream", "NNTK_REC_STREAM", &NntkOptions::rec_stream},
    {"rec_fused2", "NNTK_REC_FUSED2", &NntkOptions::rec_fused2},
    {"rec_rr", "NNTK_REC_RR", &NntkOptions::rec_rr},
    {"rec_xf", "NNTK_REC_XF", &NntkOptions::rec_xf},
    {"rec_fk", "NNTK_REC_FK", &NntkOptions::rec_fk},
    {"rec_hf", "NNTK_REC_HF", &NntkOptions::rec_hf},
    {"rec_hf_pend", "NNTK_REC_HF_PEND", &NntkOptions::rec_hf_pend},
    {"rec_bd", "NNTK_REC_BD", &NntkOptions::rec_bd},
    {"dense_frag3", "NNTK_DENSE_FRAG3", &NntkOptions::dense_frag3},
    {"dense_f16x2", "NNTK_DENSE_F16X2", &NntkOptions::dense_f16x2},
    {"train_bptt", "NNTK_TRAIN_BPTT", &NntkOptions::train_bptt},
    {"train_outer_plain", "NNTK_TRAIN_OUTER_PLAIN", &NntkOptions::train_outer_plain},
    {"spec_ppw", "NNTK_SPEC_PPW", &NntkOptions::spec_ppw},
    {"spec_variant", "NNTK_SPEC_VARIANT", &NntkOptions::spec_variant},
#ifdef NNTK_VARIANT_SPEC_DMA
    {"spec_dma", "NNTK_SPEC_DMA", &NntkOptions::spec_dma},
#endif
    {"bn_fast", "NNTK_BN_FAST", &NntkOptions::bn_fast},
    {"gemm_tm_batch", "NNTK_GEMM_TM_BATCH", &NntkOptions::gemm_tm_batch},
    {"gemm_split_bf16", "NNTK_GEMM_SPLIT_BF16", &NntkOptions::gemm_split_bf16},
    {"conv_store", "NNTK_CONV_STORE", &NntkOptions::conv_store},
    {"conv_frag3_out", "NNTK_CONV_FRAG3_OUT", &NntkOptions::conv_frag3_out},
    {"conv_flatk", "NNTK_CONV_FLATK", &NntkOptions::conv_flatk},
    {"conv_a4", "NNTK_CONV_A4", &NntkOptions::conv_a4},
    {"gemm_wide", "NNTK_GEMM_WIDE", &NntkOptions::gemm_wide},
    {"conv_dbg", "NNTK_CONV_DBG", &NntkOptions::conv_dbg},
    {"weights_check", "NNTK_WEIGHTS_CHECK", &NntkOptions::weights_check},
};
static void opt_init() {
    for (const OptDesc &d : g_opt_table) {
        const char *e = getenv(d.env);
        if (e && *e && strcmp(e, "auto") != 0 && strcmp(e, "default") != 0) g_opt.*(d.field) = atoi(e);
    }
}
const NntkOptions &nntk_options() {
    std::call_once(g_opt_once, opt_init);
    return g_opt;
}

struct ProfSpan { hipEvent_t a, b; long launches, units; int kind; hipStream_t stream; };
static std::vector<ProfSpan> g_spans;
static std::mutex g_span_mutex;
static std::atomic<bool> g_prof{false};

int nntk_prof_span_begin(int kind) {
    if (!g_prof.load(std::memory_order_relaxed)) return -1;
    ProfSpan s;
    s.launches = 0;
    s.units = 0;
    s.kind = kind;
    s.stream = t_stream;
    if (hipEventCreate(&s.a) != hipSuccess || hipEventCreate(&s.b) != hipSuccess) return -1;
    (void)hipEventRecord(s.a, t_stream);
    std::lock_guard<std::mutex> lk(g_span_mutex);
    g_spans.push_back(s);
    return (int)g_spans.size() - 1;
}
void nntk_prof_span_end(int idx, long launches, long units) {
    std::lock_guard<std::mutex> lk(g_span_mutex);
    if (idx < 0 || idx >= (int)g_spans.size()) return;
// ... 63 lines not shown
    g_persist_mutex.unlock();
}

int nntk_cu_count() {
    static std::atomic<int> cus[64];
    int dev = 0;
    if (hipGetDevice(&dev) != hipSuccess || dev < 0 || dev >= 64) return 0;
    int c = cus[dev].load(std::memory_order_relaxed);
    if (c == 0) {
        (void)hipDeviceGetAttribute(&c, hipDeviceAttributeMultiprocessorCount, dev);
        cus[dev].store(c, std::memory_order_relaxed);
    }
    return c;
}
int nntk_set_max_dynamic_lds(const void *kernel, size_t bytes) {
    struct Seen { const void *k; size_t bytes; int dev; };
    static std::vector<Seen> seen;
    static std::mutex m;
    int dev = 0;
    (void)hipGetDevice(&dev);
    std::lock_guard<std::mutex> lk(m);
    for (const Seen &s : seen)
        if (s.k == kernel && s.dev == dev && s.bytes >= bytes) return 0;
    hipError_t e = hipFuncSetAttribute(kernel, hipFuncAttributeMaxDynamicSharedMemorySize, (int)bytes);
    if (e != hipSuccess) return nntk_fail("hipFuncSetAttribute(MaxDynamicSharedMemorySize)", e);
    seen.push_back({kernel, bytes, dev});
    return 0;
}

int nntk_resident_blocks(const void *kernel, int threads, size_t lds, int max_per_cu) {
    struct Seen { const void *k; size_t lds; int dev, threads, per_cu; };
    static std::vector<Seen> seen;
    static std::mutex m;
    int dev = 0;
    if (hipGetDevice(&dev) != hipSuccess) { (void)hipGetLastError(); return 0; }
    int per_cu = -1;
    {
        std::lock_guard<std::mutex> lk(m);
        for (const Seen &s : seen)
            if (s.k == kernel && s.dev == dev && s.lds == lds && s.threads == threads) { per_cu = s.per_cu; break; }
    }
    if (per_cu < 0) {
        int n = 0;
        if (hipOccupancyMaxActiveBlocksPerMultiprocessor(&n, kernel, threads, lds) != hipSuccess) { (void)hipGetLastError(); n = 0; }
        per_cu = n;
        std::lock_guard<std::mutex> lk(m);
        seen.push_back({kernel, lds, dev, threads, per_cu});
    }
    if (per_cu > max_per_cu) per_cu = max_per_cu;
    return per_cu * nntk_cu_count();
}

static thread_local const char *t_last_rec_kernel = "";
void nntk_set_last_rec_kernel(const char *name) { t_last_rec_kernel = name; }
static thread_local const char *t_last_conv_kernel = "";
void nntk_set_last_conv_kernel(const char *name) { t_last_conv_kernel = name; }

extern "C" {

int nntk_shim_set_option(const char *name, const char *value) {
    if (!name || !value) return nntk_fail_msg("nntk_hip_set_option: NULL name or value");
    (void)nntk_options();
    std::lock_guard<std::mutex> lk(g_opt_mutex);
    for (const OptDesc &d : g_opt_table)
        if (strcmp(d.name, name) == 0) {
            g_opt.*(d.field) = (strcmp(value, "auto") == 0 || strcmp(value, "default") == 0) ? NntkOptions().*(d.field) : atoi(value);
            if (d.field == &NntkOptions::rec_persistent && g_opt.rec_persistent != 0) g_persistent_off.store(0);
            return 0;
        }
    return nntk_fail_msg("nntk_hip_set_option: unknown option");
}
int nntk_shim_get_option(const char *name, int *value) {
    if (!name || !value) return nntk_fail_msg("nntk_hip_get_option: NULL argument");
    const NntkOptions &o = nntk_options();
    for (const OptDesc &d : g_opt_table)
        if (strcmp(d.name, name) == 0) { *value = o.*(d.field); return 0; }
    return nntk_fail_msg("nntk_hip_get_option: unknown option");
}

void nntk_shim_profile_enable(int on) { g_prof.store(on != 0); }
int nntk_shim_profile_get(const char *name, double *total_ms, long *launches, long *units) {
    const int kind = (name && strcmp(name, "spectrogram") == 0) ? NNTK_SPAN_SPEC : NNTK_SPAN_REC;
    *total_ms = 0.0;
    *launches = 0;
    *units = 0;
    std::lock_guard<std::mutex> lk(g_span_mutex);
    std::vector<ProfSpan> keep;
    for (auto &s : g_spans) {
        if (s.kind != kind) { keep.push_back(s); continue; }
        float ms = 0.f;
        if (hipEventSynchronize(s.b) == hipSuccess && hipEventElapsedTime(&ms, s.a, s.b) == hipSuccess) {
            *total_ms += ms;
            *launches += s.launches;
            *units += s.units;
        }
        (void)hipEventDestroy(s.a);
        (void)hipEventDestroy(s.b);
    }
    g_spans.swap(keep);
    return 0;
}

const char *nntk_shim_error(void) { return g_err; }
void nntk_shim_set_error(const char *msg) { snprintf(g_err, sizeof(g_err), "%s", msg ? msg : ""); }
void nntk_shim_clear_error(void) { g_err[0] = 0; }

int nntk_shim_device_count(void) {
    int n = 0;
    if (hipGetDeviceCount(&n) != hipSuccess) return 0;
    return n;
}
int nntk_shim_set_device(int device) {
    NNTK_HIP_TRY(hipSetDevice(device));
    return 0;
}
const char *nntk_shim_last_rec_kernel(void) { return t_last_rec_kernel; }
const char *nntk_shim_last_conv_kernel(void) { return t_last_conv_kernel; }
int nntk_shim_get_device(void) {
    int dev = -1;
    if (hipGetDevice(&dev) != hipSuccess) { (void)hipGetLastError(); return -1; }
    return dev;
}
void nntk_shim_set_stream(void *stream) { t_stream = (hipStream_t)stream; }
void *nntk_shim_get_stream(void) { return (void *)t_stream; }
int nntk_shim_synchronize(void) {
    NNTK_HIP_TRY(hipStreamSynchronize(t_stream));
    return post_sync();
}
int nntk_shim_take_fault(void) { return fault_take() ? 1 : 0; }
int nntk_shim_persistent_disabled(void) { return nntk_persistent_disabled(); }
int nntk_shim_device_status(void) { return (t_fault_host && t_fault_host[0]) ? 1 : 0; }

void *nntk_shim_malloc(size_t bytes) {
    void *p = nullptr;
    if (bytes == 0) bytes = 16;
    hipError_t e = hipMalloc(&p, bytes);
    if (e != hipSuccess) { nntk_fail("hipMalloc", e); return nullptr; }
    return p;
}
void nntk_shim_free(void *p) {
    if (!p) return;
    nntk_shim_weights_exact_only(p, 0);
    (void)hipFree(p);
}

void *nntk_shim_host_alloc(size_t bytes) {
    void *p = nullptr;
    if (bytes == 0) bytes = 16;
    hipError_t e = hipHostMalloc(&p, bytes, hipHostMallocDefault);
    if (e != hipSuccess) { nntk_fail("hipHostMalloc", e); return nullptr; }
    memset(p, 0, bytes);
    return p;
}
void nntk_shim_host_free(void *p) { if (p) (void)hipHostFree(p); }

int nntk_shim_upload(void *d_dst, const void *h_src, size_t bytes) {
    if (!bytes) return 0;
    NNTK_HIP_TRY(hipMemcpyAsync(d_dst, h_src, bytes, hipMemcpyHostToDevice, t_stream));
    NNTK_HIP_TRY(hipStreamSynchronize(t_stream));
    return 0;
}
int nntk_shim_download_rows(void *h_dst, const void *d_src, size_t spitch, size_t width, size_t height) {
    if (!width || !height) return 0;
    NNTK_HIP_TRY(hipMemcpy2DAsync(h_dst, width, d_src, spitch, width, height, hipMemcpyDeviceToHost, t_stream));
    NNTK_HIP_TRY(hipStreamSynchronize(t_stream));
    return post_sync();
}
int nntk_shim_copy_rows_d2d(void *d_dst, const void *d_src, size_t spitch, size_t width, size_t height) {
    if (!width || !height) return 0;
// ... 373 lines not shown
```

nntoolkitcore_amd/csrc/host/recurrent.c:

```c
#include <stdarg.h>
#include <stdio.h>
#include <math.h>
#include <stdlib.h>
#include <string.h>
#include <time.h>
#include "nntk_internal.h"

#define NNTK_STREAM_MAX_T 32

RecurrentConfig RecurrentConfigCreate(int input_feature_channels, int output_feature_channels,
                                      bool return_sequences, int timesteps) {
    RecurrentConfig c;
    memset(&c, 0, sizeof(c));
    c.input_feature_channels = input_feature_channels;
    c.output_feature_channels = output_feature_channels;
    c.return_sequences = return_sequences;
    c.timesteps = timesteps;
    return c;
}


typedef struct {
    int G;
    int in, H, T;
    bool return_sequences;
    RecurrentWeights *weights;
    nntk_wblock wb;
    float *d_wp, *d_bi, *d_ut, *d_bh;
    float *d_wt;
    int wt_valid;
    int rr_exact_only;
    float *d_rr4;
    float *d_rr;
    int rr_valid;
    float *d_rr_hf;
    int rr_hf_valid;
    float hf_wscale;
    float *d_b4, *d_b4_train;
    float *d_rr_train;
    float *d_h[2], *d_c[2];
    int cur;
    float *pin_in, *pin_out;
    size_t pin_in_n, pin_out_n;
    unsigned *d_done;
    volatile unsigned *flag;
    unsigned seq;
    nntk_devbuf d_in, d_out, d_xw, d_work, d_work_rr, d_rr_stage;
    nntk_devbuf d_h2;
    nntk_devbuf d_hseq;
    nntk_devbuf d_xf3;
    nntk_devbuf d_len;
    nntk_devbuf d_bd, d_bd_len;
} rec_core;

typedef struct {
    int on, mini_batch, have_batch;
    const float *d_x_cur;
    nntk_devbuf d_x, d_h, d_Zg, d_hU, d_dxW, d_dhU, d_work, d_raw, d_grad, d_scr, d_dout, d_dX;
    nntk_train_vl vl;
    nntk_devbuf d_len, d_xm;
    nntk_devbuf d_s0;
    nntk_devbuf d_st;
    nntk_devbuf d_yo;
    float *want_hT, *want_cT;
    int bd_role, bd_merge;
    const void *bd_peer;
    nntk_devbuf d_bd_o, d_bd_do, d_bd_dx;
    nntk_devbuf d_bd_g;
    nntk_devbuf d_bd_xr;
    nntk_devbuf d_bd_host;
} rec_train;

typedef struct {
    rec_core core;
    rec_train train;
    int use_bh;
    int n_act;
    ActivationFunction act[5];
    int acts[5];
    float scales[5];
} rec_layer;
struct GRUStruct { rec_layer l; };
struct LSTMStruct { rec_layer l; };
struct RNNStruct { rec_layer l; };

#define REC_ENTER(who, handles_ok) do { nntk_shim_clear_error(); if (!(handles_ok)) NNTK_FAIL(who ": NULL handle"); } while (0)

__attribute__((format(printf, 2, 3))) static int rec_fail(const char *who, const char *fmt, ...) {
    char msg[256];
// ... 21 lines not shown

static int *stage_lengths(nntk_devbuf *buf, const int *lengths, int B, int T, int bd) {
    const int Bp = 64 * ((B + 63) / 64), rows = bd ? 2 * Bp : B, tiles = (rows + 63) / 64;
    int *hl = (int *)calloc((size_t)rows + tiles, sizeof(int));
    if (!hl) { nntk_set_error("out of host memory"); return NULL; }
    for (int v = 0; v < rows; ++v) {
        const int r = bd ? v % Bp : v;
        hl[v] = r < B ? (lengths ? lengths[r] : T) : 0;
        if (hl[v] > hl[rows + v / 64]) hl[rows + v / 64] = hl[v];
    }
    int *d_len = (int *)nntk_devbuf_reserve(buf, (size_t)rows + tiles);
    if (d_len && nntk_shim_upload_ints(d_len, hl, (long)rows + tiles)) d_len = NULL;
    free(hl);
    return d_len;
}

__attribute__((optimize("O3"))) static int rr_unsplittable(const float *v, size_t n) {
    const unsigned *u = (const unsigned *)v;
    unsigned bad = 0;
    for (size_t i = 0; i < n; ++i) {
        const unsigned a = u[i] & 0x7fffffffu;
        bad |= (unsigned)(a > 0x7f7f0000u) | (unsigned)(a - 1u < 0x007fffffu);
    }
    return bad != 0;
}

static int core_init(rec_core *c, int G, RecurrentConfig base) {
    memset(c, 0, sizeof(*c));
    c->G = G;
    c->in = base.input_feature_channels;
    c->H = base.output_feature_channels;
    c->T = base.timesteps;
    c->return_sequences = base.return_sequences;
    size_t w = (size_t)c->in * G * c->H, u = (size_t)c->H * G * c->H, b = (size_t)G * c->H;
    if (nntk_wblock_init(&c->wb, w + u + 2 * b)) return -1;
    c->weights = (RecurrentWeights *)malloc(sizeof(RecurrentWeights));
    c->weights->W = c->wb.host;
    c->weights->U = c->weights->W + w;
    c->weights->b_i = c->weights->U + u;
    c->weights->b_h = c->weights->b_i + b;
    size_t hs = ((size_t)c->H + 63) & ~(size_t)63;
    float *st = (float *)nntk_shim_malloc(4 * hs * sizeof(float));
    if (!st) return -1;
    c->d_h[0] = st; c->d_h[1] = st + hs; c->d_c[0] = st + 2 * hs; c->d_c[1] = st + 3 * hs;
    c->cur = 0;
    if (nntk_shim_memset(st, 0, 4 * hs * sizeof(float))) return -1;
    return 0;
}

static void core_free(rec_core *c) {
    nntk_shim_synchronize();
    nntk_shim_free(c->d_wp); nntk_shim_free(c->d_bi); nntk_shim_free(c->d_ut); nntk_shim_free(c->d_bh); nntk_shim_free(c->d_wt);
    nntk_shim_free(c->d_rr_hf);
    nntk_shim_free(c->d_rr); nntk_shim_free(c->d_rr4); nntk_shim_free(c->d_rr_train); nntk_shim_free(c->d_b4); nntk_shim_free(c->d_b4_train);
    nntk_shim_free(c->d_h[0]);
    nntk_shim_host_free(c->pin_in); nntk_shim_host_free(c->pin_out); nntk_shim_host_free((void *)c->flag);
    nntk_shim_free(c->d_done);
    nntk_devbuf_free(&c->d_in); nntk_devbuf_free(&c->d_out); nntk_devbuf_free(&c->d_xw); nntk_devbuf_free(&c->d_work); nntk_devbuf_free(&c->d_work_rr); nntk_devbuf_free(&c->d_rr_stage);
    nntk_devbuf_free(&c->d_hseq); nntk_devbuf_free(&c->d_xf3); nntk_devbuf_free(&c->d_h2);
    nntk_devbuf_free(&c->d_len);
    nntk_devbuf_free(&c->d_bd); nntk_devbuf_free(&c->d_bd_len);
    nntk_wblock_free(&c->wb);
    free(c->weights);
}

static void train_free(rec_train *t) {
    nntk_devbuf_free(&t->d_x); nntk_devbuf_free(&t->d_h); nntk_devbuf_free(&t->d_Zg); nntk_devbuf_free(&t->d_hU);
    nntk_devbuf_free(&t->d_dxW); nntk_devbuf_free(&t->d_dhU); nntk_devbuf_free(&t->d_work); nntk_devbuf_free(&t->d_raw);
    nntk_devbuf_free(&t->d_grad); nntk_devbuf_free(&t->d_scr); nntk_devbuf_free(&t->d_dout); nntk_devbuf_free(&t->d_dX);
    nntk_devbuf_free(&t->d_len); nntk_devbuf_free(&t->d_xm); nntk_devbuf_free(&t->d_s0); nntk_devbuf_free(&t->d_st);
    nntk_devbuf_free(&t->d_yo);
    nntk_devbuf_free(&t->d_bd_o); nntk_devbuf_free(&t->d_bd_do); nntk_devbuf_free(&t->d_bd_dx); nntk_devbuf_free(&t->d_bd_xr);
    nntk_devbuf_free(&t->d_bd_host); nntk_devbuf_free(&t->d_bd_g);
}

static rec_layer *layer_create(int G, RecurrentConfig base, int use_bh, const ActivationFunction *act, int n_act) {
    nntk_shim_clear_error();
    rec_layer *l = (rec_layer *)calloc(1, sizeof(rec_layer));
    if (!l) return NULL;
    l->use_bh = use_bh;
    l->n_act = n_act;
    memcpy(l->act, act, (size_t)n_act * sizeof(*act));
    if (core_init(&l->core, G, base)) { free(l); return NULL; }
    return l;
}
static void layer_train_on(rec_layer *l, RecurrentTrainingConfig training_config) {
    l->train.on = 1;
    l->train.mini_batch = training_config.mini_batch_size;
}
static void layer_destroy(rec_layer *l) {
    if (!l) return;
    core_free(&l->core);
    train_free(&l->train);
    free(l);
}

static float *pack_gate_transposed(const float *src, int G, int H, size_t *n) {
    const int Hj_p = (H + 15) & ~15, Hk_p = (H + 31) & ~31;
    *n = (size_t)G * Hj_p * Hk_p;
    float *tmp = (float *)calloc(*n, sizeof(float));
    if (!tmp) { nntk_set_error("out of host memory while packing recurrent weights"); return NULL; }
    for (int k = 0; k < H; ++k)
        for (int g = 0; g < G; ++g)
            for (int j = 0; j < H; ++j)
                tmp[((size_t)g * Hj_p + j) * Hk_p + k] = src[(size_t)k * G * H + (size_t)g * H + j];
    return tmp;
}

static int core_upload(rec_core *c) {
    int G = c->G, H = c->H;
    if (nntk_upload_gemm_weights(&c->d_wp, c->weights->W, c->in, G * H)) return -1;
    if (nntk_upload_floats(&c->d_bi, c->weights->b_i, (size_t)G * H)) return -1;
    if (nntk_upload_floats(&c->d_bh, c->weights->b_h, (size_t)G * H)) return -1;
    size_t n;
    float *tmp = pack_gate_transposed(c->weights->U, G, H, &n);
    if (!tmp) return -1;
    int rc = nntk_upload_floats(&c->d_ut, tmp, n);
    free(tmp);
    if (rc) return rc;
    c->wt_valid = 0;
    c->rr_valid = 0;
    c->rr_hf_valid = 0;
    c->rr_exact_only = rr_unsplittable(c->weights->W, (size_t)c->in * G * H + (size_t)H * G * H);
    nntk_wblock_mark_uploaded(&c->wb);
    return 0;
}

static int core_ensure_wt(rec_core *c) {
    if (c->wt_valid) return 0;
    if (c->in != c->H) NNTK_FAIL("fused GRU stack: layer 2's input size must equal its hidden size");
    size_t n;
    float *tmp = pack_gate_transposed(c->weights->W, c->G, c->H, &n);
    if (!tmp) return -1;
    int rc = nntk_upload_floats(&c->d_wt, tmp, n);
    free(tmp);
    if (rc) return rc;
    c->wt_valid = 1;
    return 0;
}

static int core_ensure(rec_core *c, int check_edits) {
    if (nntk_wblock_dirty(&c->wb, check_edits)) return core_upload(c);
    return 0;
}

static int core_reset_state(rec_core *c) {
    size_t hs = ((size_t)c->H + 63) & ~(size_t)63;
    c->cur = 0;
    return nntk_shim_memset(c->d_h[0], 0, 4 * hs * sizeof(float));
}

static int core_broadcast(rec_core *c, int root) {
    if (nntk_shim_dist_broadcast_host(c->wb.host, c->wb.n, root)) return -1;
    return core_upload(c);
}
static int core_sync(rec_core *c) {
    nntk_shim_synchronize();
    return core_upload(c);
}
static int core_load_device(rec_core *c, const char *who, const float *d_block) {
    if (!d_block) return rec_fail(who, "NULL block");
    if (nntk_shim_download(c->wb.host, d_block, c->wb.n * sizeof(float))) return -1;
    return core_upload(c);
}

static int gate_kind(ActivationFunction a, int *kind, float *scale) {
    if (!a) NNTK_FAIL("recurrent layer: NULL gate activation");
    if (!nntk_act_fusable(a))
        NNTK_FAIL("recurrent layer: gate activations must be built-in identity/sigmoid/tanh/relu "
                  "(custom host callbacks and softmax cannot run inside the device step kernel)");
    *kind = a->kind;
    *scale = a->kind == NNTK_ACT_RELU ? a->relu_a : 1.0f;
    return 0;
}
static int layer_acts(rec_layer *l) {
// ... 105 lines not shown
    const int H = c->H, in = c->in;
    const float *sW = c->wb.shadow, *sU = sW + (size_t)in * 3 * H, *sbi = sU + (size_t)H * 3 * H, *sbh = sbi + 3 * (size_t)H;
    return gru_rr_build_image(in, H, sW, sU, sbi, sbh, &c->d_rr, nntk_shim_rr_image_floats_xf(H, in), &c->d_b4, &c->d_rr_stage, &c->d_rr4);
}
static int layer_rr_images(rec_layer *l) {
    rec_core *c = &l->core;
    if (nntk_shim_fk_image_floats(c->H, c->in) && !c->d_rr4) c->rr_valid = 0;
    if (c->rr_valid) return 0;
    if (c->G == 4 ? lstm_rr_images(c) : gru_rr_images(c)) return -1;
    c->rr_valid = 1;
    return 0;
}

static int core_try_rr(rec_layer *l, const rr_io *io, int B, int stateful) {
    rec_core *c = &l->core;
    if (stateful && rr_option() != 1) return 1;
    if (!layer_takes_rr(l)) return 1;
    const float *xf3 = NULL;
    const int xm = rr_input(c, io, B, &xf3);
    if (xm < 0) return -1;
    if (xm == 2) return 1;
    if (layer_rr_images(l)) return -1;
    float *d_work = nntk_devbuf_reserve(&c->d_work_rr, nntk_shim_lstm_rr_work_floats(B, c->H));
    float *d_hseq = io->d_out_f3 ? io->d_out_f3 : nntk_devbuf_reserve(&c->d_hseq, nntk_shim_rr_hseq_floats(B, c->T, c->H));
    if (!d_work || !d_hseq) return -1;
    const int gru = c->G == 3;
    const float *x = xm ? NULL : io->d_in, *xf = xm ? xf3 : NULL;
    const float *bi = gru ? c->d_b4 : c->d_bi, *bh = !gru && l->use_bh ? c->d_bh : NULL;
    if (io->d_len)
        return nntk_shim_rr_varlen(gru, x, xf, c->d_rr, c->d_rr4, bi, bh, io->d_h0, io->d_c0, io->d_out, d_hseq, io->d_hT, io->d_cT, d_work,
                                   io->d_len, B, c->T, c->in, c->H, c->return_sequences);
    const float *h0 = stateful ? c->d_h[c->cur] : NULL, *c0 = stateful ? c->d_c[c->cur] : NULL;
    float *hT = stateful ? c->d_h[c->cur ^ 1] : NULL, *cT = stateful ? c->d_c[c->cur ^ 1] : NULL;
    if (gru)
        return nntk_shim_gru_rr(x, xf, c->d_rr, c->d_rr4, bi, h0, io->d_out, d_hseq, hT, d_work, B, c->T, c->in, c->H, c->return_sequences, 0, 0);
    return nntk_shim_lstm_rr(x, xf, c->d_rr, c->d_rr4, bi, bh, h0, c0, io->d_out, io->d_out_h2, d_hseq, hT, cT, d_work, B, c->T, c->in, c->H,
                             c->return_sequences);
}

static const char *core_plan(rec_layer *l, char *buf, size_t n) {
    const rec_core *c = &l->core;
    const char *cell = c->G == 4 ? "lstm" : c->G == 3 ? "gru" : "rnn";
    if (layer_acts(l)) return c->G == 4 ? "lstm: invalid gate activations" : "gru: invalid gate activations";
    const char *why = rr_why_not(l, c->wb.uploaded && c->rr_exact_only, nntk_shim_rr_image_floats_xf(c->H, c->in) != 0);
    if (why)
        snprintf(buf, n, "%s: exact-f32 kernels (projection GEMM + rec_persistent_kernel, per-timestep kernels when that does not fit) -- %s", cell, why);
    else if (nntk_shim_fk_image_floats(c->H, c->in) != 0)
        snprintf(buf, n, "%s: %s_fk_kernel<16,%d,%d> (register-resident split-bf16 x 3 without split-K, input projection fused; the input is packed into frag3 form first); the stateful single-sequence call keeps the exact-f32 kernels",
                 cell, cell, c->in <= 128 ? 8 : 16, 4);
    else
        snprintf(buf, n, "%s: %s_rr_kernel<%d,%d> (register-resident split-bf16 x 3, input projection fused)%s; the stateful single-sequence call keeps the exact-f32 kernels",
                 cell, cell, c->H <= 256 ? 4 : 8, c->in <= 64 ? 1 : c->in <= 128 ? 2 : 4,
                 nntk_shim_lstm_rr_image_floats(c->H, c->in) != 0 ? "" : "; in % 8 != 0: the input is packed into frag3 form first");
    return buf;
}


static int core_apply_device(rec_layer *l, const float *d_in, float *d_out, int B, int stateful) {
    rec_core *c = &l->core;
    int G = c->G, H = c->H, T = c->T;
    if (B <= 0 || T <= 0) return 0;
    const rr_io io = { .d_in = d_in, .d_out = d_out };
    int rc = core_try_rr(l, &io, B, stateful);
    if (rc <= 0) return rc;
    float *d_xw = nntk_devbuf_reserve(&c->d_xw, (size_t)T * B * G * H);
    float *d_work = nntk_devbuf_reserve(&c->d_work, nntk_shim_recurrent_work_floats(B, H));
    if (!d_xw || !d_work) return -1;
    if (nntk_shim_conv1d(d_in, c->d_wp, c->d_bi, NULL, 0.f, NNTK_ACT_IDENTITY, 1.f, d_xw,
                         B, T, c->in, G * H, 1, 1, T, 1))
        return -1;
    const float *bh = l->use_bh ? c->d_bh : NULL;
    const float *h0 = stateful ? c->d_h[c->cur] : NULL, *c0 = stateful ? c->d_c[c->cur] : NULL;
    float *hT = stateful ? c->d_h[c->cur ^ 1] : NULL, *cT = stateful ? c->d_c[c->cur ^ 1] : NULL;
    if (G == 1)
        return nntk_shim_rnn(d_xw, c->d_ut, bh, h0, d_out, hT, d_work, B, T, H, c->return_sequences, l->acts[0], l->scales[0]);
    if (G == 4)
        return nntk_shim_lstm(d_xw, c->d_ut, bh, h0, c0, d_out, hT, cT, d_work, B, T, H, c->return_sequences, l->acts, l->scales);
    return nntk_shim_gru(d_xw, c->d_ut, bh, h0, d_out, hT, d_work, B, T, H, c->return_sequences, l->acts, l->scales);
}

static int core_apply_device_vl(rec_layer *l, const char *who, const float *d_in, float *d_out, int B, const int *lengths,
                                const float *d_h0, const float *d_c0, float *d_hT, float *d_cT) {
    rec_core *c = &l->core;
    const int G = c->G, H = c->H, T = c->T;
    if (B < 0) return rec_fail(who, "batch %d < 0", B);
    int T_min, T_max;
    if (nntk_check_lengths(who, lengths, B, T, &T_min, &T_max)) return -1;
    if (B == 0 || T <= 0) return 0;
    const int *d_len = stage_lengths(&c->d_len, lengths, B, T, 0);
    if (!d_len) return -1;
    if (G != 4) d_c0 = NULL, d_cT = NULL;
    const int zero_pad = c->return_sequences && T_min < T;
    const rr_io io = { .d_in = d_in, .d_out = d_out, .d_len = d_len, .d_h0 = d_h0, .d_c0 = d_c0, .d_hT = d_hT, .d_cT = d_cT };
    const int rc = core_try_rr(l, &io, B, 0);
    if (rc < 0) return -1;
    if (rc == 0) return zero_pad ? nntk_shim_varlen_zero_pad(d_out, d_len, B, T, H) : 0;
    float *d_xw = nntk_devbuf_reserve(&c->d_xw, (size_t)T * B * G * H);
    float *d_work = nntk_devbuf_reserve(&c->d_work, nntk_shim_recurrent_work_floats(B, H));
    if (!d_xw || !d_work) return -1;
    if (T_max > 0 && nntk_shim_conv1d(d_in, c->d_wp, c->d_bi, NULL, 0.f, NNTK_ACT_IDENTITY, 1.f, d_xw, B, T, c->in, G * H, 1, 1, T, 1))
        return -1;
    if (nntk_shim_rec_varlen(G, d_xw, c->d_ut, l->use_bh ? c->d_bh : NULL, d_h0, d_c0, d_out, d_hT, d_cT,
                             d_work, B, T, H, c->return_sequences, l->acts, l->scales, d_len, T_max))
        return -1;
    return zero_pad ? nntk_shim_varlen_zero_pad(d_out, d_len, B, T, H) : 0;
}
// ... 1123 lines not shown
    static _Thread_local char buf[320];
    return filter ? core_plan(&filter->l, buf, sizeof buf) : "";
}

int LSTMApplyInference(LSTM filter, const float *input, float *output) {
    REC_ENTER("LSTMApplyInference", filter);
    return layer_apply_inference(&filter->l, "LSTMApplyInference", input, output);
}
int LSTMApplyInferenceBatch(LSTM filter, const float *input, float *output, int batch) {
    REC_ENTER("LSTMApplyInferenceBatch", filter);
    return layer_apply_batch(&filter->l, input, output, batch);
}
int LSTMApplyDevice(LSTM filter, const float *d_input, float *d_output, int batch) {
    REC_ENTER("LSTMApplyDevice", filter);
    return layer_apply_device(&filter->l, d_input, d_output, batch);
}
int LSTMApplyDeviceVarLen(LSTM filter, const float *d_input, float *d_output, int batch, const int *lengths,
                          const float *d_h0, const float *d_c0, float *d_hT, float *d_cT) {
    REC_ENTER("LSTMApplyDeviceVarLen", filter);
    return layer_apply_device_vl(&filter->l, "LSTMApplyDeviceVarLen", d_input, d_output, batch, lengths, d_h0, d_c0, d_hT, d_cT);
}
int LSTMApplyInferenceBatchVarLen(LSTM filter, const float *input, float *output, int batch, const int *lengths,
                                  const float *h0, const float *c0, float *hT, float *cT) {
    REC_ENTER("LSTMApplyInferenceBatchVarLen", filter);
    return layer_apply_host_vl(&filter->l, "LSTMApplyInferenceBatchVarLen", input, output, batch, lengths, h0, c0, hT, cT);
}
int LSTMApplyDeviceFrag3(LSTM filter, const float *d_input, const float *d_input_frag3, float *d_output, float *d_output_frag3, int batch) {
    REC_ENTER("LSTMApplyDeviceFrag3", filter);
    return layer_apply_device_f3(&filter->l, d_input, d_input_frag3, d_output, d_output_frag3, batch);
}
int LSTMBidirectionalApplyDevice(LSTM forward, LSTM backward, const float *d_input, float *d_output, int batch, const int *lengths, int merge) {
    REC_ENTER("LSTMBidirectionalApplyDevice", forward && backward);
    return layer_apply_bd(&forward->l, &backward->l, "LSTMBidirectionalApplyDevice", d_input, d_output, batch, lengths, merge);
}
int LSTMBidirectionalApplyInferenceBatch(LSTM forward, LSTM backward, const float *input, float *output, int batch, const int *lengths, int merge) {
    REC_ENTER("LSTMBidirectionalApplyInferenceBatch", forward && backward);
    return layer_apply_bd_host(&forward->l, &backward->l, "LSTMBidirectionalApplyInferenceBatch", input, output, batch, lengths, merge);
}

static int lstm_try_rr_hf(rec_layer *l, const float *d_in, const float *d_in_f3, float *d_out_h2, int B) {
    rec_core *c = &l->core;
    if (rr_why_not(l, c->rr_exact_only, nntk_shim_lstm_rr_hf_ok(c->H, c->in))) return 1;
    if (!c->rr_hf_valid) {
        const size_t nW = (size_t)c->in * 4 * c->H, nU = (size_t)c->H * 4 * c->H;
        float us = nntk_f16_scale(c->weights->U, nU), mw = 0.f;
        for (size_t i = 0; i < nW; ++i) { float a = fabsf(c->weights->W[i]); if (a > mw) mw = a; }
        c->hf_wscale = (us > 0.f && us < 1e15f && us > 1e-15f && mw * 32768.f * us < 1e30f) ? 32768.f * us : 0.f;
        if (c->hf_wscale > 0.f) {
            size_t img = nntk_shim_lstm_rr_hf_image_floats(c->H, c->in);
            if (!c->d_rr_hf && !(c->d_rr_hf = (float *)nntk_shim_malloc(img * sizeof(float)))) return -1;
            if (nntk_shim_lstm_rr_pack_hf(c->d_ut, c->d_wp, c->d_rr_hf, c->H, c->in, us, c->hf_wscale)) return -1;
        }
        c->rr_hf_valid = 1;
    }
    if (!(c->hf_wscale > 0.f)) return 1;
    const float *xf3 = d_in_f3;
    if (!xf3) {
        float *buf = nntk_devbuf_reserve(&c->d_xf3, nntk_shim_frag3_floats(B, c->T, c->in));
        if (!buf || nntk_shim_frag3_pack(d_in, buf, B, c->T, c->in)) return -1;
        xf3 = buf;
    }
    float *d_work = nntk_devbuf_reserve(&c->d_work_rr, nntk_shim_lstm_rr_work_floats(B, c->H));
    if (!d_work) return -1;
    return nntk_shim_lstm_rr_hf(xf3, c->d_rr_hf, c->d_bi, l->use_bh ? c->d_bh : NULL, d_out_h2, d_work, B, c->T, c->in, c->H, 1.f / c->hf_wscale);
}
static int lstm_apply_device_h2(LSTM filter, const float *d_in, const float *d_in_f3, float *d_out_h2, int B) {
    rec_layer *l = &filter->l;
    rec_core *c = &l->core;
    if (layer_acts(l)) return -1;
    if (!layer_std_acts(l) || !c->return_sequences) return 1;
    if (B <= 0 || c->T <= 0) return 0;
    if (core_ensure(c, 0)) return -1;
    int rc = lstm_try_rr_hf(l, d_in, d_in_f3, d_out_h2, B);
    if (rc <= 0) return rc;
    if (!nntk_shim_fk_image_floats(c->H, c->in)) {
        const rr_io io = { .d_in = d_in, .d_in_f3 = d_in_f3, .d_out_h2 = d_out_h2 };
        rc = core_try_rr(l, &io, B, 0);
        if (rc <= 0) return rc;
    }
    float *o = nntk_devbuf_reserve(&c->d_out, (size_t)B * c->T * c->H);
    if (!o) return -1;
    if (core_apply_device_f3(l, d_in, d_in_f3, o, NULL, B)) return -1;
    return nntk_shim_frag2h_pack(o, d_out_h2, B, c->T, c->H);
}
int LSTMApplyDeviceFrag2h(LSTM filter, const float *d_input, const float *d_input_frag3, float *d_output_frag2h, int batch) {
    nntk_shim_clear_error();
    if (!filter || (!d_input && !d_input_frag3) || !d_output_frag2h) NNTK_FAIL("LSTMApplyDeviceFrag2h: NULL argument");
    int rc = lstm_apply_device_h2(filter, d_input, d_input_frag3, d_output_frag2h, batch);
    if (rc == 1) NNTK_FAIL("LSTMApplyDeviceFrag2h: the frag2h form holds |h| < 2 -- standard activations and return_sequences only");
    return rc;
}
int nntk_lstm_apply_device_h2(LSTM filter, const float *d_in, const float *d_in_f3, float *d_out_h2, int B) {
    return lstm_apply_device_h2(filter, d_in, d_in_f3, d_out_h2, B);
}
float *nntk_lstm_frag2h_scratch(LSTM f, int batch) {
    return nntk_devbuf_reserve(&f->l.core.d_h2, nntk_shim_frag2h_floats(batch, f->l.core.T, f->l.core.H));
}
void nntk_lstm_dims(LSTM f, int *T, int *in, int *H, int *return_sequences) {
    const rec_core *c = &f->l.core;
    *T = c->T; *in = c->in; *H = c->H; *return_sequences = c->return_sequences ? 1 : 0;
}
float *nntk_lstm_frag3_scratch(LSTM f, int batch) {
    rec_core *c = &f->l.core;
    size_t a = nntk_shim_rr_hseq_floats(batch, c->T, c->H), b = nntk_shim_frag3_floats(batch, c->T, c->H);
    return nntk_devbuf_reserve(&c->d_hseq, a > b ? a : b);
}

int LSTMApplyTrainingBatch(LSTM filter, const float *input, float *output) {
    REC_ENTER("LSTMApplyTrainingBatch", filter);
    return train_apply_host(&filter->l, "LSTMApplyTrainingBatch", input, output);
}
int LSTMApplyTrainingBatchDevice(LSTM filter, const float *d_input, float *d_output) {
    REC_ENTER("LSTMApplyTrainingBatchDevice", filter);
    return train_apply_dev(&filter->l, "LSTMApplyTrainingBatchDevice", d_input, d_output);
}
void LSTMCalculateGradient(LSTM filter, LSTMGradient *gradient, float *d_out) {
    REC_ENTER_GRADIENT("LSTMCalculateGradient", filter && gradient && d_out);
// ... 167 lines not shown
```

nntoolkitcore_amd/csrc/host/runtime.c:

```c
#include <math.h>
#include <stdlib.h>
#include <string.h>
#include "nntk_internal.h"

void nntk_set_error(const char *msg) { nntk_shim_set_error(msg); }

int nntk_hip_device_count(void) { return nntk_shim_device_count(); }
int nntk_hip_set_device(int device) { return nntk_shim_set_device(device); }
void nntk_hip_set_stream(void *hip_stream) { nntk_shim_set_stream(hip_stream); }
void *nntk_hip_get_stream(void) { return nntk_shim_get_stream(); }
int nntk_hip_synchronize(void) { return nntk_shim_synchronize(); }
const char *nntk_last_error(void) { return nntk_shim_error(); }
void nntk_hip_profile_enable(int on) { nntk_shim_profile_enable(on); }
int nntk_hip_profile_get(const char *name, double *total_ms, long *launches, long *timesteps) {
    return nntk_shim_profile_get(name, total_ms, launches, timesteps);
}
const char *nntk_version(void) { return "nntoolkitcore_hip 0.2 (gfx950)"; }
int nntk_hip_set_option(const char *name, const char *value) { nntk_shim_clear_error(); return nntk_shim_set_option(name, value); }
int nntk_hip_get_option(const char *name, int *value) { nntk_shim_clear_error(); return nntk_shim_get_option(name, value); }
int nntk_hip_device_status(void) { return nntk_shim_device_status(); }
const char *nntk_hip_last_recurrent_kernel(void) { return nntk_shim_last_rec_kernel(); }
const char *nntk_hip_last_conv_kernel(void) { return nntk_shim_last_conv_kernel(); }

int nntk_dist_get_unique_id(unsigned char id[NNTK_DIST_ID_BYTES]) { nntk_shim_clear_error(); return nntk_shim_dist_unique_id(id); }
int nntk_dist_init(const unsigned char id[NNTK_DIST_ID_BYTES], int rank, int world_size) { nntk_shim_clear_error(); return nntk_shim_dist_init(id, rank, world_size); }
int nntk_dist_rank(void) { return nntk_shim_dist_rank(); }
int nntk_dist_world_size(void) { return nntk_shim_dist_world(); }
int nntk_dist_broadcast(float *host_block, size_t n_floats, int root) { nntk_shim_clear_error(); return nntk_shim_dist_broadcast_host(host_block, n_floats, root); }
int nntk_dist_barrier(void) { nntk_shim_clear_error(); return nntk_shim_dist_barrier(); }
int nntk_dist_allreduce(float *host_block, size_t n_floats) { nntk_shim_clear_error(); return nntk_shim_dist_allreduce_host(host_block, n_floats); }
int nntk_dist_allreduce_device(float *d_block, size_t n_floats) { nntk_shim_clear_error(); return nntk_shim_dist_allreduce_device(d_block, n_floats); }
int nntk_dist_finalize(void) { nntk_shim_clear_error(); return nntk_shim_dist_finalize(); }
void nntk_dist_shard_range(int n_utterances, int world_size, int rank, int *lo, int *hi) {
    int base = n_utterances / world_size, rem = n_utterances % world_size;
    *lo = rank * base + (rank < rem ? rank : rem);
    *hi = *lo + base + (rank < rem ? 1 : 0);
}

float *nntk_device_alloc(size_t n_floats) { return (float *)nntk_shim_malloc(n_floats * sizeof(float)); }
void nntk_device_free(float *ptr) { nntk_shim_free(ptr); }
int nntk_device_upload(float *dst_device, const float *src_host, size_t n_floats) {
    return nntk_shim_upload(dst_device, src_host, n_floats * sizeof(float));
}
int nntk_device_download(float *dst_host, const float *src_device, size_t n_floats) {
    return nntk_shim_download(dst_host, src_device, n_floats * sizeof(float));
}

size_t nntk_frag3_floats(int batch, int T, int C) { return nntk_shim_frag3_floats(batch, T, C); }
int nntk_frag3_pack_device(const float *d_x, float *d_frag3, int batch, int T, int C) {
    nntk_shim_clear_error();
    if (!d_x || !d_frag3) NNTK_FAIL("nntk_frag3_pack_device: NULL argument");
    return nntk_shim_frag3_pack(d_x, d_frag3, batch, T, C);
}
size_t nntk_frag2h_floats(int batch, int T, int C) { return nntk_shim_frag2h_floats(batch, T, C); }
int nntk_frag2h_pack_device(const float *d_x, float *d_frag2h, int batch, int T, int C) {
    nntk_shim_clear_error();
    if (!d_x || !d_frag2h) NNTK_FAIL("nntk_frag2h_pack_device: NULL argument");
    return nntk_shim_frag2h_pack(d_x, d_frag2h, batch, T, C);
}
int nntk_frag2h_unpack_device(const float *d_frag2h, float *d_x, int batch, int T, int C) {
    nntk_shim_clear_error();
    if (!d_x || !d_frag2h) NNTK_FAIL("nntk_frag2h_unpack_device: NULL argument");
    return nntk_shim_frag2h_unpack(d_frag2h, d_x, batch, T, C);
}
int nntk_frag3_unpack_device(const float *d_frag3, float *d_x, int batch, int T, int C) {
    nntk_shim_clear_error();
    if (!d_x || !d_frag3) NNTK_FAIL("nntk_frag3_unpack_device: NULL argument");
    return nntk_shim_frag3_unpack(d_frag3, d_x, batch, T, C);
}

int nntk_wblock_init(nntk_wblock *wb, size_t n_floats) {
    wb->n = n_floats;
    wb->uploaded = 0;
    wb->host = (float *)nntk_shim_host_alloc(n_floats * sizeof(float));
// ... 132 lines not shown
```

Measured before the change: 74.17 million.

## Add split-f16 (two-piece) recurrent-state path to the fused LSTM fk kernel

Extends the fused fk recurrent kernel with an HF mode. The hidden-state recurrence uses two-piece f16 splits (hi/lo) instead of three-piece bf16 splits, which cuts MFMA count, state publish stores and ring traffic per timestep. The host side packs and caches a separate fk image and passes it to the hf launch path, plus a detail-name query for diagnostics. The new rec_hf_fk option defaults to 0 and rec_hf_pend changes from 1 to -1, so whether the new path runs by default depends on option handling not shown. Trades some accuracy for less work on the serial recurrence.

```diff
diff --git a/include/nntoolkitcore_hip.h b/include/nntoolkitcore_hip.h
--- a/include/nntoolkitcore_hip.h
+++ b/include/nntoolkitcore_hip.h
@@ -296,6 +296,7 @@
 int         nntk_hip_get_option(const char *name, int *value);
 int         nntk_hip_device_status(void);
 const char *nntk_hip_last_recurrent_kernel(void);
+const char *nntk_hip_last_recurrent_detail(void);
 const char *nntk_hip_last_conv_kernel(void);
 void        nntk_hip_profile_enable(int on);
 int         nntk_hip_profile_get(const char *name, double *total_ms, long *launches, long *timesteps);
diff --git a/nntoolkitcore_amd/capi.py b/nntoolkitcore_amd/capi.py
--- a/nntoolkitcore_amd/capi.py
+++ b/nntoolkitcore_amd/capi.py
@@ -279,6 +279,7 @@
     "nntk_hip_get_option": (C.c_int, [C.c_char_p, C.POINTER(C.c_int)]),
     "nntk_hip_device_status": (C.c_int, []),
     "nntk_hip_last_recurrent_kernel": (C.c_char_p, []),
+    "nntk_hip_last_recurrent_detail": (C.c_char_p, []),
     "nntk_hip_last_conv_kernel": (C.c_char_p, []),
     "nntk_hip_profile_enable": (None, [C.c_int]),
     "nntk_hip_profile_get": (C.c_int, [C.c_char_p, C.POINTER(C.c_double), C.POINTER(C.c_long), C.POINTER(C.c_long)]),
diff --git a/nntoolkitcore_amd/csrc/hip/nntk_common.hpp b/nntoolkitcore_amd/csrc/hip/nntk_common.hpp
--- a/nntoolkitcore_amd/csrc/hip/nntk_common.hpp
+++ b/nntoolkitcore_amd/csrc/hip/nntk_common.hpp
@@ -22,7 +22,8 @@
     int rec_xf = -1;
     int rec_fk = -1;
     int rec_hf = -1;
-    int rec_hf_pend = 1;
+    int rec_hf_pend = -1;
+    int rec_hf_fk = 0;
     int rec_bd = -1;
     int dense_frag3 = -1;
     int dense_f16x2 = -1;
@@ -55,6 +56,7 @@
 int nntk_cu_count();
 void nntk_set_last_conv_kernel(const char *name);
 void nntk_set_last_rec_kernel(const char *name);
+void nntk_set_last_rec_detail(const char *name);
 int nntk_set_max_dynamic_lds(const void *kernel, size_t bytes);
 int nntk_outer_mfma_launch(const float *d_A, const float *d_B, float *d_partial, long rows, int I, int K, int a_shift_T,
                            long rps, long seq_pitch, long row_pitch);
diff --git a/nntoolkitcore_amd/csrc/hip/nntk_shim.h b/nntoolkitcore_amd/csrc/hip/nntk_shim.h
--- a/nntoolkitcore_amd/csrc/hip/nntk_shim.h
+++ b/nntoolkitcore_amd/csrc/hip/nntk_shim.h
@@ -33,6 +33,7 @@
 int nntk_shim_take_fault(void);
 int nntk_shim_persistent_disabled(void);
 const char *nntk_shim_last_conv_kernel(void);
+const char *nntk_shim_last_rec_detail(void);
 const char *nntk_shim_last_rec_kernel(void);
 int nntk_shim_device_status(void);
 
@@ -257,8 +258,12 @@
 int nntk_shim_lstm_rr_hf_ok(int H, int in);
 size_t nntk_shim_lstm_rr_hf_image_floats(int H, int in);
 int nntk_shim_lstm_rr_pack_hf(const float *d_ut, const float *d_wp, float *d_img, int H, int in, float uscale, float wscale);
-int nntk_shim_lstm_rr_hf(const void *d_xf3, const float *d_img, const float *d_bi, const float *d_bh, float *d_h2, float *d_work,
+int nntk_shim_lstm_rr_hf(const void *d_xf3, const float *d_img, const float *d_imgfk, const float *d_bi, const float *d_bh, float *d_h2, float *d_work,
                          int B, int T, int in, int H, float z_scale);
+int nntk_shim_fk_hf_ok(int H, int in);
+size_t nntk_shim_fk_hf_image_floats(int H, int in);
+int nntk_shim_fk_pack_hf(const float *d_ut, const float *d_wp, float *d_img, int H, int in, float uscale, float wscale);
+const char *nntk_shim_fk_hf_kernel_name(void);
 
 size_t nntk_shim_frag3_floats(int B, int T, int C);
 int nntk_shim_frag3_pack(const float *d_x, void *d_frag, int B, int T, int C);
diff --git a/nntoolkitcore_amd/csrc/hip/recurrent_fk.hip b/nntoolkitcore_amd/csrc/hip/recurrent_fk.hip
--- a/nntoolkitcore_amd/csrc/hip/recurrent_fk.hip
+++ b/nntoolkitcore_amd/csrc/hip/recurrent_fk.hip
@@ -43,7 +43,7 @@
 #define FK_FINE_OUT(gs, t) do {} while (0)
 #endif
 
-__host__ __device__ inline int fk_blocks_per_ct(int NKH, int NKX, int NW) { return NW * (NKH * 3 + NKX * 3); }
+__host__ __device__ inline int fk_blocks_per_ct(int NKH, int NKX, int NW, int NH = 3) { return NW * (NKH * NH + NKX * 3); }
 __host__ __device__ inline int fk_nmr(int NKH) { return NKH <= 16 ? 3 : 2; }
 __host__ __device__ inline int fk_nmw(int NKX, int NW) { return NW == 4 && NKX > 8 ? 1 : 0; }
 __host__ __device__ inline int fk_walk(int NGP, int NW, int ct, int ug, int pos) {
@@ -54,9 +54,10 @@
 template <bool RAW>
 __global__ __launch_bounds__(256) void fk_pack_kernel(const float *__restrict__ ut, const float *__restrict__ wp,
                                                       rr_v4u *__restrict__ img, int H, int in, int Hj_p, int Hk_p, int Kin_p,
-                                                      int NKH, int NKX, int NMR, int NW, int NCT) {
+                                                      int NKH, int NKX, int NMR, int NW, int NCT, float uscale = 0.0f, float wscale = 1.0f) {
+    const bool hf = uscale > 0.0f;
     const int NMW = fk_nmw(NKX, NW);
-    const int n_ur = NW * NKH * NMR, n_wr = NW * NKX * NMW, n_ul = NW * NKH * (3 - NMR), bpc = fk_blocks_per_ct(NKH, NKX, NW);
+    const int n_ur = NW * NKH * NMR, n_wr = NW * NKX * NMW, n_ul = hf ? 0 : NW * NKH * (3 - NMR), bpc = fk_blocks_per_ct(NKH, NKX, NW, hf ? 2 : 3);
     const long total = (long)NCT * bpc * 64;
     for (long e = blockIdx.x * (long)blockDim.x + threadIdx.x; e < total; e += (long)gridDim.x * blockDim.x) {
         const int l = (int)(e & 63);
@@ -89,15 +90,29 @@
             v[q] = val;
         }
         rr_v4u hi, mid, lo;
+        if (hf) {
+            if (part == 0) {
+                unsigned h4[4], l4[4];
+#pragma unroll
+                for (int q = 0; q < 4; ++q) rr_split_pair_f16(v[2 * q] * uscale, v[2 * q + 1] * uscale, h4[q], l4[q]);
+                img[e] = m == 0 ? (rr_v4u){h4[0], h4[1], h4[2], h4[3]} : (rr_v4u){l4[0], l4[1], l4[2], l4[3]};
+                continue;
+            }
+#pragma unroll
+            for (int q = 0; q < 8; ++q) v[q] *= wscale;
+        }
         rr_split8(v, hi, mid, lo);
         img[e] = m == 0 ? hi : m == 1 ? mid : lo;
     }
 }
 
-template <int NKH, int NKX, int CELL, int NW, int ND, bool VL = false, bool BD = false>
+template <int NKH, int NKX, int CELL, int NW, int ND, bool VL = false, bool BD = false, bool HF = false>
 __device__ __forceinline__ void fk_body(const RRParams &p) {
     static_assert(!BD || VL, "BD: per-row lengths");
-    constexpr int NMR = NKH <= 16 ? 3 : 2;
+    static_assert(!HF || (CELL == 0 && NW == 4 && !VL && !BD), "HF: the LSTM on 32 rows x 32 units, whole batch rows");
+    constexpr int NH = HF ? 2 : 3;
+    constexpr int NMR = HF ? 2 : NKH <= 16 ? 3 : 2;
+    constexpr int NUL = NH - NMR;
     constexpr int NMW = NW == 4 && NKX > 8 ? 1 : 0;
     constexpr int FK_RING = fk_ring(NKX, NW);
     constexpr bool BURST = FK_RING == 2;
@@ -115,7 +130,7 @@
     constexpr int FIN_G = NW == 4 ? 1 : (NGX >= 4 ? 4 : NGX);
     extern __shared__ __attribute__((aligned(16))) char smem[];
     rr_v4u *ULs = reinterpret_cast<rr_v4u *>(smem);
-    rr_v4u *WXs = ULs + NW * NKH * (3 - NMR) * 64;
+    rr_v4u *WXs = ULs + NW * NKH * NUL * 64;
     rr_v4u *ring = WXs + NW * NKX * (3 - NMW) * 64;
     unsigned *flg = reinterpret_cast<unsigned *>(ring + 4 * FK_RING * 3 * 64);
 #define FK_FENCE() asm volatile("" ::: "memory")
@@ -144,7 +159,7 @@
     }
     const bool grp_ok = 8 * gi < H;
 
-    const rr_v4u *img = (bwd ? p.img_b : p.img) + (size_t)ct * fk_blocks_per_ct(NKH, NKX, NW) * 64;
+    const rr_v4u *img = (bwd ? p.img_b : p.img) + (size_t)ct * fk_blocks_per_ct(NKH, NKX, NW, NH) * 64;
     rr_bf16x8 uh[NKH][NMR];
 #pragma unroll
     for (int pos = 0; pos < NKH; ++pos)
@@ -164,7 +179,7 @@
     }
     {
         const rr_v4u *src = img + (size_t)(NW * NKH * NMR + NW * NKX * NMW) * 64;
-        constexpr int n16 = (NW * NKH * (3 - NMR) + NW * NKX * (3 - NMW)) * 64;
+        constexpr int n16 = (NW * NKH * NUL + NW * NKX * (3 - NMW)) * 64;
         for (int e = tid; e < n16; e += 256) ULs[e] = src[e];
         for (int e = tid; e < 4 * FK_RING * 64; e += 256) flg[e] = 0u;
     }
@@ -207,7 +222,7 @@
     };
     const int lane16 = lane * 16;
     const int ugh = (ug ^ (ct / NGH)) & (NW - 1), ugx = (ug ^ (ct / NGX)) & (NW - 1);
-    const int hso = ht_abs * NKS * 3 * 1024;
+    const int hso = ht_abs * NKS * NH * 1024;
     const int xso = ht_abs * p.NKSx * 3 * 1024;
     const int ldo = BD ? p.ldo : H;
     const long o_row_bytes = (long)(p.return_sequences ? p.T : 1) * ldo * 4;
@@ -216,7 +231,7 @@
         (void *)((bwd ? p.out_b : p.out) + (size_t)rb0 * (o_row_bytes / 4)), 0, (int)(o_range < 0x7fffffffL ? o_range : 0x7fffffffL), 0x00020000);
     const bool row_ok = hf * 32 + n < rows_valid && grp_ok;
     const int out_vo = row_ok ? (int)((hf * 32 + n) * o_row_bytes) + jf * 4 : 0x7fff0000;
-    const int pub_vo = grp_ok ? ((ht_abs * NKS + (gi >> 1)) * 3) * 1024 + (32 * (gi & 1) + n) * 16 + 8 * kh : RR_OOB_F;
+    const int pub_vo = grp_ok ? ((ht_abs * NKS + (gi >> 1)) * NH) * 1024 + (32 * (gi & 1) + n) * 16 + 8 * kh : RR_OOB_F;
     RR_BARRIER();
 
     using Tt = std::true_type;
@@ -234,10 +249,10 @@
         if (is_h) {
             const __amdgpu_buffer_rsrc_t rs = rs_rd(tq);
             const int ks = NW * ((g_h + ct) % NGH) + ugh;
-            const int so = hso + ks * 3072;
+            const int so = hso + ks * NH * 1024;
             const int vo = lane16 + (ks < NKS ? 0 : RR_OOB_F);
 #pragma unroll
-            for (int m = 0; m < 3; ++m) {
+            for (int m = 0; m < NH; ++m) {
                 if (m < m0 || m >= m1) continue;
                 S[si][m] = __builtin_amdgcn_raw_buffer_load_b128(rs, vo + m * 1024, so, 16 );
                 RR_BOUND(tq ? 3 : 4, tq ? (size_t)(tq - 1) * p.hstep : 0, vo + m * 1024, so, tq < T ? hb_bytes : 0, 16);
@@ -258,7 +273,7 @@
     auto probe = [&](int si) __attribute__((always_inline)) {
         unsigned mx = 0;
 #pragma unroll
-        for (int m = 0; m < 3; ++m) {
+        for (int m = 0; m < NH; ++m) {
             const rr_v4u v = S[si][m];
             mx = max(mx, max(max(v.x, v.y), max(v.z, v.w)));
         }
@@ -279,12 +294,12 @@
             if (expired && lane == 0) __hip_atomic_fetch_or(p.fault, 1u, __ATOMIC_RELAXED, __HIP_MEMORY_SCOPE_AGENT);
         }
     };
-    auto ring_put = [&](int si, int slot, unsigned seq, int piece) __attribute__((always_inline)) {
+    auto ring_put = [&](int si, int slot, unsigned seq, int piece, int nf = 3) __attribute__((always_inline)) {
         rr_v4u *d = ring + ((w * FK_RING + slot) * 3) * 64 + lane;
         FK_FENCE();
 #pragma unroll
         for (int m = 0; m < 3; ++m)
-            if (piece < 0 || piece == m) d[m * 64] = S[si][m];
+            if ((piece < 0 || piece == m) && m < nf) d[m * 64] = S[si][m];
         FK_FENCE();
         if (piece < 0 || piece == 2) flg[(w * FK_RING + slot) * 64 + lane] = seq;
         FK_FENCE();
@@ -295,16 +310,16 @@
         fl[j - 1] = flg[(pw * FK_RING + slot) * 64 + lane];
         FK_FENCE();
     };
-    auto ring_data = [&](int j, int slot, int m0, int m1) __attribute__((always_inline)) {
+    auto ring_data = [&](int j, int slot, int m0, int m1, int nf = 3) __attribute__((always_inline)) {
         const int pw = hf * NW + (ug ^ j);
         const rr_v4u *s = ring + ((pw * FK_RING + slot) * 3) * 64 + lane;
         FK_FENCE();
 #pragma unroll
         for (int m = 0; m < 3; ++m)
-            if (m >= m0 && m < m1) P[j - 1][m] = s[m * 64];
+            if (m >= m0 && m < m1 && m < nf) P[j - 1][m] = s[m * 64];
         FK_FENCE();
     };
-    auto ring_check = [&](int slot, unsigned seq) __attribute__((always_inline)) {
+    auto ring_check = [&](int slot, unsigned seq, int nf) __attribute__((always_inline)) {
         bool bad = false;
 #pragma unroll
         for (int j = 1; j < NW; ++j) bad |= fl[j - 1] != seq;
@@ -322,7 +337,7 @@
             }
             if (expired && lane == 0) __hip_atomic_fetch_or(p.fault, 1u, __ATOMIC_RELAXED, __HIP_MEMORY_SCOPE_AGENT);
 #pragma unroll
-            for (int j = 1; j < (BURST ? NW : 2); ++j) ring_data(j, slot, 0, 3);
+            for (int j = 1; j < (BURST ? NW : 2); ++j) ring_data(j, slot, 0, 3, nf);
         }
     };
     float hn[4];
@@ -331,7 +346,7 @@
         if (RR_DBG(2)) return;
         float zc[4];
 #pragma unroll
-        for (int g = 0; g < 4; ++g) zc[g] = acc[4 * g + e] + bsum[g][e];
+        for (int g = 0; g < 4; ++g) zc[g] = HF ? fmaf(acc[4 * g + e], p.z_scale, bsum[g][e]) : acc[4 * g + e] + bsum[g][e];
         if (RR_DBG(64)) { hn[e] = zc[0] + zc[1] + zc[2] + zc[3] + cst[e]; return; }
         if (CELL == 1) {
             const float zg = nntk_fast_sigmoid(zc[0]);
@@ -359,6 +374,20 @@
     };
     auto fin_store = [&](int t) __attribute__((always_inline)) {
         if (RR_DBG(2)) return;
+        if constexpr (HF) {
+            if (!RR_DBG(128)) {
+                unsigned sh0, sl0, sh1, sl1;
+                rr_split_pair_h2(hn[0], hn[1], sh0, sl0);
+                rr_split_pair_h2(hn[2], hn[3], sh1, sl1);
+                const fk_v2u a = {(unsigned)min(sh0, 0xfffffffeu), (unsigned)min(sh1, 0xfffffffeu)};
+                const fk_v2u b = {(unsigned)min(sl0, 0xfffffffeu), (unsigned)min(sl1, 0xfffffffeu)};
+                const __amdgpu_buffer_rsrc_t rs = rs_wr(t);
+                __builtin_amdgcn_raw_buffer_store_b64(a, rs, pub_vo, 0, RR_ST_AUX );
+                __builtin_amdgcn_raw_buffer_store_b64(b, rs, pub_vo + 1024, 0, RR_ST_AUX);
+                RR_BOUND(3, (size_t)t * p.hstep, pub_vo + 1024, 0, hb_bytes, 8);
+            }
+            return;
+        }
         if (!RR_DBG(128)) {
             unsigned sh0, sm0, sl0, sh1, sm1, sl1;
             rr_split_pair(hn[0], hn[1], sh0, sm0, sl0);
@@ -389,14 +418,14 @@
         const fk_v2u pend = {RR_PENDING, RR_PENDING};
         __builtin_amdgcn_raw_buffer_store_b64(pend, rs2, vo2, 0, RR_ST_AUX);
         __builtin_amdgcn_raw_buffer_store_b64(pend, rs2, vo2 + 1024, 0, RR_ST_AUX);
-        __builtin_amdgcn_raw_buffer_store_b64(pend, rs2, vo2 + 2048, 0, RR_ST_AUX);
-        RR_BOUND(3, (size_t)(t + 1 < T ? t + 1 : t) * p.hstep, vo2 + 2048, 0, hb_bytes, 8);
+        if (NH == 3) __builtin_amdgcn_raw_buffer_store_b64(pend, rs2, vo2 + 2048, 0, RR_ST_AUX);
+        RR_BOUND(3, (size_t)(t + 1 < T ? t + 1 : t) * p.hstep, vo2 + (NH - 1) * 1024, 0, hb_bytes, 8);
     };
 
     constexpr int PA[6] = {0, 2, 1, 0, 1, 0}, PB[6] = {2, 0, 1, 1, 0, 0};
     auto lds_fetch_a = [&](bool is_h, int pos, int buf) __attribute__((always_inline)) {
         if (is_h) {
-            if (NMR == 2) ulo[buf] = __builtin_bit_cast(rr_bf16x8, ULs[(ug * NKH + pos) * 64 + lane]);
+            if (NUL == 1) ulo[buf] = __builtin_bit_cast(rr_bf16x8, ULs[(ug * NKH + pos) * 64 + lane]);
         } else {
 #pragma unroll
             for (int m = NMW; m < 3; ++m) wa[buf][m] = __builtin_bit_cast(rr_bf16x8, WXs[((ug * NKX + pos) * (3 - NMW) + (m - NMW)) * 64 + lane]);
@@ -404,6 +433,18 @@
     };
     auto mult = [&](f32x16 &acc, bool is_h, int pos, int buf, const rr_v4u (&bsrc)[3], int j0, int j1) __attribute__((always_inline)) {
         if (RR_DBG(16)) return;
+        if constexpr (HF) {
+            if (is_h) {
+                constexpr int QA[3] = {0, 1, 0}, QB[3] = {1, 0, 0};
+#pragma unroll
+                for (int pr = 0; pr < 6; pr += 2) {
+                    if (pr < j0 || pr >= j1) continue;
+                    acc = __builtin_amdgcn_mfma_f32_32x32x16_f16(__builtin_bit_cast(rr_f16x8, uh[pos][QA[pr / 2]]),
+                                                                 __builtin_bit_cast(rr_f16x8, bsrc[QB[pr / 2]]), acc, 0, 0, 0);
+                }
+                return;
+            }
+        }
         rr_bf16x8 b[3];
 #pragma unroll
         for (int m = 0; m < 3; ++m) b[m] = __builtin_bit_cast(rr_bf16x8, bsrc[m]);
@@ -411,7 +452,7 @@
         for (int pr = 0; pr < 6; ++pr) {
             if (pr < j0 || pr >= j1) continue;
             rr_bf16x8 av;
-            if (is_h) av = (NMR == 2 && PA[pr] == 2) ? ulo[buf] : uh[pos][PA[pr] < NMR ? PA[pr] : 0];
+            if (is_h) av = (NUL == 1 && PA[pr] == 2) ? ulo[buf] : uh[pos][PA[pr] < NMR ? PA[pr] : 0];
             else av = PA[pr] < NMW ? wr[NMW ? pos : 0][NMW ? PA[pr] : 0] : wa[buf][PA[pr]];
             acc = __builtin_amdgcn_mfma_f32_32x32x16_bf16(av, b[PB[pr]], acc, 0, 0, 0);
         }
@@ -442,6 +483,7 @@
             const int q1 = (gs + 1) % NG, t1 = t + (gs + 1 >= NG ? 1 : 0);
             const bool h1 = q1 < NGH;
             f32x16 &a = is_h ? acc : accn;
+            const int nf = HF && is_h ? 2 : 3, nf1 = HF && h1 ? 2 : 3;
             FK_STAMP(t, gs);
             if (gs == NGH) {
 #pragma unroll
@@ -461,13 +503,14 @@
             if (chk1) { const rr_v4u v = S[si1][0]; mx0 = max(max(v.x, v.y), max(v.z, v.w)); asm volatile("" : "+v"(mx0)); }
             FK_PIN();
             mult(a, is_h, pos0, 0, S[si], 1, 2); FK_PIN();
-            ring_data(1, slot, 0, 3);
-            if (BURST && NW == 4) ring_data(2, slot, 0, 3);
+            ring_data(1, slot, 0, 3, nf);
+            if (BURST && NW == 4) ring_data(2, slot, 0, 3, nf);
             if (chk1) { const rr_v4u v = S[si1][1]; mx1 = max(mx0, max(max(v.x, v.y), max(v.z, v.w))); asm volatile("" : "+v"(mx1)); }
             FK_PIN();
             mult(a, is_h, pos0, 0, S[si], 2, 3); FK_PIN();
-            if (BURST && NW == 4) ring_data(3, slot, 0, 3);
-            if (chk1) { const rr_v4u v = S[si1][2]; mx2 = max(mx1, max(max(v.x, v.y), max(v.z, v.w))); asm volatile("" : "+v"(mx2)); }
+            if (BURST && NW == 4) ring_data(3, slot, 0, 3, nf);
+            if (chk1 && NH == 3) { const rr_v4u v = S[si1][2]; mx2 = max(mx1, max(max(v.x, v.y), max(v.z, v.w))); asm volatile("" : "+v"(mx2)); }
+            else mx2 = mx1;
             lds_fetch_a(is_h, pos0 + 1, 1); FK_PIN();
             FK_FINE(gs, 1);
             {
@@ -480,20 +523,20 @@
                 if (t1 <= 0) pend = 0ull;
                 if (__builtin_expect((pend | __builtin_amdgcn_ballot_w64(bad)) != 0, 0)) {
                     if (pend != 0) settle(q1, si1, t1);
-                    if (!RR_DBG(512)) ring_check(slot, seq);
+                    if (!RR_DBG(512)) ring_check(slot, seq, nf);
                 }
             }
             FK_FINE(gs, 2);
 #ifdef FK_COARSE_GS
             if (gs == FK_COARSE_GS) FK_STAMP(t, 40);
 #endif
-            if (!RR_DBG(512) && !LATE) ring_put(si1, slot1, seq + 1u, 0);
+            if (!RR_DBG(512) && !LATE) ring_put(si1, slot1, seq + 1u, 0, nf1);
             FK_PIN();
             mult(a, is_h, pos0, 0, S[si], 3, 4); FK_PIN();
-            if (!RR_DBG(512) && !LATE) ring_put(si1, slot1, seq + 1u, 1);
+            if (!RR_DBG(512) && !LATE) ring_put(si1, slot1, seq + 1u, 1, nf1);
             FK_PIN();
             mult(a, is_h, pos0, 0, S[si], 4, 5); FK_PIN();
-            if (!RR_DBG(512) && !LATE) ring_put(si1, slot1, seq + 1u, 2);
+            if (!RR_DBG(512) && !LATE) ring_put(si1, slot1, seq + 1u, 2, nf1);
             FK_PIN();
             mult(a, is_h, pos0, 0, S[si], 5, 6); FK_PIN();
             if (HP && gs == 0) { mark_next(t); FK_PIN(); }
@@ -506,16 +549,16 @@
 #pragma unroll
             for (int j = 1; j < NW; ++j) {
                 mult(a, is_h, pos0 + j, j & 1, P[j - 1], 0, 2); if (!fin_here) FK_PIN();
-                if (j + 1 < NW && !BURST) ring_data(j + 1, slot, 0, 1);
+                if (j + 1 < NW && !BURST) ring_data(j + 1, slot, 0, 1, nf);
                 issue_sched(gs, PAR, t, j - 1, 0, 1); if (!fin_here) FK_PIN();
                 if (j + 1 < NW) lds_fetch_a(is_h, pos0 + j + 1, (j + 1) & 1);
                 else lds_fetch_a(h1, NW * (h1 ? q1 : q1 - NGH), 0);
                 if (!fin_here) FK_PIN();
                 mult(a, is_h, pos0 + j, j & 1, P[j - 1], 2, 4); if (!fin_here) FK_PIN();
-                if (j + 1 < NW && !BURST) ring_data(j + 1, slot, 1, 2);
+                if (j + 1 < NW && !BURST) ring_data(j + 1, slot, 1, 2, nf);
                 issue_sched(gs, PAR, t, j - 1, 1, 2); if (!fin_here) FK_PIN();
                 mult(a, is_h, pos0 + j, j & 1, P[j - 1], 4, 6); if (!fin_here) FK_PIN();
-                if (j + 1 < NW && !BURST) ring_data(j + 1, slot, 2, 3);
+                if (j + 1 < NW && !BURST) ring_data(j + 1, slot, 2, 3, nf);
                 issue_sched(gs, PAR, t, j - 1, 2, 3); if (!fin_here) FK_PIN();
                 FK_FINE(gs, 3 + j);
 #ifdef FK_COARSE_GS
@@ -542,7 +585,7 @@
                     const unsigned long long pend = probe(si1) | inject;
                     if (__builtin_expect(pend != 0, 0)) settle(q1, si1, t1);
                 }
-                if (!RR_DBG(512)) ring_put(si1, slot1, seq + 1u, -1);
+                if (!RR_DBG(512)) ring_put(si1, slot1, seq + 1u, -1, nf1);
             }
             __builtin_amdgcn_sched_barrier(0);
             FK_FINE_OUT(gs, t);
@@ -599,6 +642,11 @@
 __global__ __launch_bounds__(256) void lstm_fk_kernel(RRParams p) { fk_body<NKH, NKX, 0, NW, ND, VL, BD>(p); }
 template <int NKH, int NKX, int NW, int ND, bool VL = false, bool BD = false>
 __global__ __launch_bounds__(256) void gru_fk_kernel(RRParams p) { fk_body<NKH, NKX, 1, NW, ND, VL, BD>(p); }
+#ifndef FK_ND_HF
+#define FK_ND_HF 4
+#endif
+template <int NKH, int NKX, int NW, int ND>
+__global__ __launch_bounds__(256) void lstm_fk_hf_kernel(RRParams p) { fk_body<NKH, NKX, 0, NW, ND, false, false, true>(p); }
 
 static bool fk_shape(int H, int in, int *NKH, int *NKX, int *NW) {
     if ((H % 16) != 0 || H <= 128 || H > 256 || in <= 64 || in > 256) return false;
@@ -612,8 +660,13 @@
 #endif
     return true;
 }
-static size_t fk_lds_bytes(int NKH, int NKX, int NW) {
-    return (size_t)(NW * NKH * (3 - fk_nmr(NKH)) + NW * NKX * (3 - fk_nmw(NKX, NW)) + 4 * fk_ring(NKX, NW) * 3) * 1024 + 4 * fk_ring(NKX, NW) * 64 * 4;
+static bool fk_shape_hf(int H, int in, int *NKH, int *NKX, int *NW) {
+    if ((H % 16) != 0 || H <= 256 || H > 512 || in < 1 || in > 128) return false;
+    *NKH = 32; *NKX = 8; *NW = 4;
+    return true;
+}
+static size_t fk_lds_bytes(int NKH, int NKX, int NW, bool hf = false) {
+    return (size_t)(NW * NKH * (hf ? 0 : 3 - fk_nmr(NKH)) + NW * NKX * (3 - fk_nmw(NKX, NW)) + 4 * fk_ring(NKX, NW) * 3) * 1024 + 4 * fk_ring(NKX, NW) * 64 * 4;
 }
 extern "C" size_t nntk_shim_fk_image_floats(int H, int in) {
     int NKH, NKX, NW;
@@ -638,13 +691,43 @@
 extern "C" int nntk_shim_fk_pack(const float *d_ut, const float *d_wp, float *d_img, int H, int in) { return fk_pack(false, d_ut, d_wp, d_img, H, in); }
 extern "C" int nntk_shim_fk_pack_raw(const float *d_U, const float *d_W, float *d_img, int H, int in) { return fk_pack(true, d_U, d_W, d_img, H, in); }
 
-int nntk_fk_launch(RRParams q, const float *d_imgfk, const float *d_imgfk_b, int cell, size_t *launches) {
+extern "C" int nntk_shim_fk_hf_ok(int H, int in) {
     int NKH, NKX, NW;
-    if (!d_imgfk || !q.xf3 || q.x_tm || q.out_tm || !fk_shape(q.H, q.in, &NKH, &NKX, &NW)) return 1;
+    const NntkOptions &o = nntk_options();
+    return fk_shape_hf(H, in, &NKH, &NKX, &NW) && o.rec_hf != 0 && o.rec_hf_fk > 0 && o.rec_hf_pend < 0;
+}
+extern "C" const char *nntk_shim_fk_hf_kernel_name(void) { return "lstm_fk_hf_kernel<32,8,4," NNTK_STR(FK_ND_HF) ">"; }
+extern "C" size_t nntk_shim_fk_hf_image_floats(int H, int in) {
+    int NKH, NKX, NW;
+    if (!fk_shape_hf(H, in, &NKH, &NKX, &NW)) return 0;
+    return (size_t)((H + 8 * NW - 1) / (8 * NW)) * fk_blocks_per_ct(NKH, NKX, NW, 2) * 256;
+}
+extern "C" int nntk_shim_fk_pack_hf(const float *d_ut, const float *d_wp, float *d_img, int H, int in, float uscale, float wscale) {
+    int NKH, NKX, NW;
+    if (!fk_shape_hf(H, in, &NKH, &NKX, &NW) || !(uscale > 0.0f)) return nntk_fail_msg("fk_pack_hf: shape / scale not taken by the full-K HF kernel");
+    const int Hj_p = (H + 15) & ~15, Hk_p = (H + 31) & ~31;
+    int Kin_p, N_p;
+    nntk_shim_conv_pack_sizes(in, 4 * H, 1, &Kin_p, &N_p);
+    const int NCT = (H + 8 * NW - 1) / (8 * NW);
+    const long total = (long)NCT * fk_blocks_per_ct(NKH, NKX, NW, 2) * 64;
+    long g = (total + 255) / 256;
+    if (g > 4096) g = 4096;
+    hipLaunchKernelGGL(fk_pack_kernel<false>, dim3((unsigned)g), dim3(256), 0, nntk_stream(), d_ut, d_wp, (rr_v4u *)d_img, H, in, Hj_p, Hk_p, Kin_p, NKH, NKX, 2, NW, NCT,
+                       uscale, wscale);
+    NNTK_LAUNCH_CHECK("fk_pack_kernel");
+    return 0;
+}
+
+int nntk_fk_launch(RRParams q, const float *d_imgfk, const float *d_imgfk_b, int cell, size_t *launches, bool hf) {
+    int NKH, NKX, NW;
+    if (!d_imgfk || !q.xf3 || q.x_tm || q.out_tm) return 1;
+    if (hf ? !nntk_shim_fk_hf_ok(q.H, q.in) || !fk_shape_hf(q.H, q.in, &NKH, &NKX, &NW) : !fk_shape(q.H, q.in, &NKH, &NKX, &NW)) return 1;
     const bool bd = q.out_b != nullptr;
     if (bd && (!d_imgfk_b || !q.len)) return 1;
+    if (hf && (bd || q.len || cell != 0 || q.out || q.c0 || q.h0 || q.hT || q.cT || !q.return_sequences)) return 1;
     void (*kern)(RRParams) = nullptr;
-    if (bd) {
+    if (hf) kern = lstm_fk_hf_kernel<32, 8, 4, FK_ND_HF>;
+    else if (bd) {
         if (cell == 1) kern = NKX == 8 ? gru_fk_kernel<16, 8, 4, FK_ND_4, true, true> : gru_fk_kernel<16, 16, 4, FK_ND_4W, true, true>;
         else kern = NKX == 8 ? lstm_fk_kernel<16, 8, 4, FK_ND_4, true, true> : lstm_fk_kernel<16, 16, 4, FK_ND_4W, true, true>;
     } else if (q.len) {
@@ -656,7 +739,7 @@
     if (NW == 2 && (q.len || bd)) return 1;
     if (NW == 2) kern = cell == 1 ? gru_fk_kernel<16, 16, 2, FK_ND_2> : lstm_fk_kernel<16, 16, 2, FK_ND_2>;
 #endif
-    const size_t lds = fk_lds_bytes(NKH, NKX, NW);
+    const size_t lds = fk_lds_bytes(NKH, NKX, NW, hf);
     if (lds > 160 * 1024) return 1;
     if (nntk_set_max_dynamic_lds((const void *)kern, lds)) return -1;
     const int NCT = (q.H + 8 * NW - 1) / (8 * NW);
@@ -676,6 +759,7 @@
     if (launches) *launches = (size_t)((nbt_total + tiles_per_launch - 1) / tiles_per_launch);
     static const char *const names[2][3] = {{"lstm_fk_kernel<16,8,4>", "lstm_fk_kernel<16,16,4>", "lstm_fk_kernel<16,16,2>"}, {"gru_fk_kernel<16,8,4>", "gru_fk_kernel<16,16,4>", "gru_fk_kernel<16,16,2>"}};
     static const char *const bd_names[2][2] = {{"lstm_fk_kernel<16,8,4,bd>", "lstm_fk_kernel<16,16,4,bd>"}, {"gru_fk_kernel<16,8,4,bd>", "gru_fk_kernel<16,16,4,bd>"}};
+    if (hf) return 0;
     nntk_set_last_rec_kernel(bd ? bd_names[cell == 1][NKX == 16] : names[cell == 1][NW == 2 ? 2 : NKX == 16]);
     return 0;
 }
diff --git a/nntoolkitcore_amd/csrc/hip/recurrent_rr.hip b/nntoolkitcore_amd/csrc/hip/recurrent_rr.hip
--- a/nntoolkitcore_amd/csrc/hip/recurrent_rr.hip
+++ b/nntoolkitcore_amd/csrc/hip/recurrent_rr.hip
@@ -819,7 +819,8 @@
     return 0;
 }
 
-int nntk_fk_launch(RRParams q, const float *d_imgfk, const float *d_imgfk_b, int cell, size_t *launches);
+int nntk_fk_launch(RRParams q, const float *d_imgfk, const float *d_imgfk_b, int cell, size_t *launches, bool hf);
+extern "C" const char *nntk_shim_fk_hf_kernel_name(void);
 struct RRIo {
     const float *img4;
     const float *x; const void *xf3; float *out; float *hseq; float *work;
@@ -886,9 +887,9 @@
     NNTK_LAUNCH_CHECK("rr_pack_kernel");
     return 0;
 }
-extern "C" int nntk_shim_lstm_rr_hf(const void *d_xf3, const float *d_img, const float *d_bi, const float *d_bh, float *d_h2, float *d_work,
+extern "C" int nntk_shim_lstm_rr_hf(const void *d_xf3, const float *d_img, const float *d_imgfk, const float *d_bi, const float *d_bh, float *d_h2, float *d_work,
                                     int B, int T, int in, int H, float z_scale) {
-    RRIo io = {nullptr, nullptr, d_xf3, nullptr, d_h2, d_work, nullptr, nullptr, nullptr, nullptr, nullptr, nullptr, 0, 0, nullptr, 1, z_scale, nullptr};
+    RRIo io = {d_imgfk, nullptr, d_xf3, nullptr, d_h2, d_work, nullptr, nullptr, nullptr, nullptr, nullptr, nullptr, 0, 0, nullptr, 1, z_scale, nullptr};
     return rr_launch(io, d_img, d_bi, d_bh, B, T, in, H, 1, 0);
 }
 extern "C" int nntk_shim_gru_rr(const float *d_x, const void *d_xf3, const float *d_img, const float *d_img4, const float *d_b4, const float *d_h0, float *d_out,
@@ -952,7 +953,7 @@
     const bool hf = io.hf != 0;
     if (!(hf ? rr_shape_hf(H, in, &KH, &KX) : rr_shape(H, in, xf, &KH, &KX))) return 1;
     if (!xf && ((((size_t)io.x) & 15) != 0 || (in % 4) != 0)) return 1;
-    if (hf && (KH != 8 || cell != 0 || !xf || train || io.h0 || io.out || io.out_h2 || io.img4 || !return_sequences || opt.rec_hf == 0)) return 1;
+    if (hf && (KH != 8 || cell != 0 || !xf || train || io.h0 || io.out || io.out_h2 || !return_sequences || opt.rec_hf == 0)) return 1;
     const int NCT = H / 16;
     if (!rr_tile_fits(T, in, bd ? io.ldo : H)) return 1;
     void (*kern)(RRParams) = nullptr;
@@ -1025,7 +1026,7 @@
     int took4 = 1;
     if (xf && !train && io.img4 && !io.out_tm) {
         q.flags = flags;
-        took4 = nntk_fk_launch(q, io.img4, io.img4_b, cell, &launches);
+        took4 = nntk_fk_launch(q, io.img4, io.img4_b, cell, &launches, hf);
         if (took4 < 0) { nntk_persistent_launch_end(); return -1; }
     }
     if (took4 == 1)
@@ -1056,7 +1057,10 @@
                                                   {{"gru_rr_kernel<4,1,bd>", "gru_rr_kernel<4,2,bd>", "gru_rr_kernel<4,4,bd>"}, {"gru_rr_kernel<8,1,bd>", "gru_rr_kernel<8,2,bd>", ""}}};
     if (bd && took4 == 1) nntk_set_last_rec_kernel(bd_names[cell == 1][KH == 8][KX == 1 ? 0 : KX == 2 ? 1 : 2]);
     else if (hf && !hfp && KX != 4) nntk_set_last_rec_kernel(KX == 2 ? "lstm_rr_kernel<8,2,flags,hf>" : "lstm_rr_kernel<8,1,flags,hf>");
-    else if (hf) nntk_set_last_rec_kernel(KX == 4 ? "lstm_rr_kernel<8,4,hf>" : KX == 2 ? "lstm_rr_kernel<8,2,hf>" : "lstm_rr_kernel<8,1,hf>");
+    else if (hf) {
+        nntk_set_last_rec_kernel(KX == 4 ? "lstm_rr_kernel<8,4,hf>" : KX == 2 ? "lstm_rr_kernel<8,2,hf>" : "lstm_rr_kernel<8,1,hf>");
+        if (took4 == 0) nntk_set_last_rec_detail(nntk_shim_fk_hf_kernel_name());
+    }
     else if (took4 == 1) nntk_set_last_rec_kernel(names[cell == 1][KH == 8][KX == 1 ? 0 : KX == 2 ? 1 : 2]);
     return 0;
 }
diff --git a/nntoolkitcore_amd/csrc/hip/runtime.hip b/nntoolkitcore_amd/csrc/hip/runtime.hip
--- a/nntoolkitcore_amd/csrc/hip/runtime.hip
+++ b/nntoolkitcore_amd/csrc/hip/runtime.hip
@@ -39,6 +39,7 @@
     {"rec_fk", "NNTK_REC_FK", &NntkOptions::rec_fk},
     {"rec_hf", "NNTK_REC_HF", &NntkOptions::rec_hf},
     {"rec_hf_pend", "NNTK_REC_HF_PEND", &NntkOptions::rec_hf_pend},
+    {"rec_hf_fk", "NNTK_REC_HF_FK", &NntkOptions::rec_hf_fk},
     {"rec_bd", "NNTK_REC_BD", &NntkOptions::rec_bd},
     {"dense_frag3", "NNTK_DENSE_FRAG3", &NntkOptions::dense_frag3},
     {"dense_f16x2", "NNTK_DENSE_F16X2", &NntkOptions::dense_f16x2},
@@ -208,7 +209,9 @@
 }
 
 static thread_local const char *t_last_rec_kernel = "";
-void nntk_set_last_rec_kernel(const char *name) { t_last_rec_kernel = name; }
+static thread_local const char *t_last_rec_detail = "";
+void nntk_set_last_rec_kernel(const char *name) { t_last_rec_kernel = name; t_last_rec_detail = ""; }
+void nntk_set_last_rec_detail(const char *name) { t_last_rec_detail = name; }
 static thread_local const char *t_last_conv_kernel = "";
 void nntk_set_last_conv_kernel(const char *name) { t_last_conv_kernel = name; }
 
@@ -271,6 +274,7 @@
     return 0;
 }
 const char *nntk_shim_last_rec_kernel(void) { return t_last_rec_kernel; }
+const char *nntk_shim_last_rec_detail(void) { return t_last_rec_detail; }
 const char *nntk_shim_last_conv_kernel(void) { return t_last_conv_kernel; }
 int nntk_shim_get_device(void) {
     int dev = -1;
diff --git a/nntoolkitcore_amd/csrc/host/recurrent.c b/nntoolkitcore_amd/csrc/host/recurrent.c
--- a/nntoolkitcore_amd/csrc/host/recurrent.c
+++ b/nntoolkitcore_amd/csrc/host/recurrent.c
@@ -34,7 +34,8 @@
     float *d_rr;
     int rr_valid;
     float *d_rr_hf;
-    int rr_hf_valid;
+    float *d_fk_hf;
+    int rr_hf_valid, fk_hf_valid;
     float hf_wscale;
     float *d_b4, *d_b4_train;
     float *d_rr_train;
@@ -162,6 +163,7 @@
     nntk_shim_synchronize();
     nntk_shim_free(c->d_wp); nntk_shim_free(c->d_bi); nntk_shim_free(c->d_ut); nntk_shim_free(c->d_bh); nntk_shim_free(c->d_wt);
     nntk_shim_free(c->d_rr_hf);
+    nntk_shim_free(c->d_fk_hf);
     nntk_shim_free(c->d_rr); nntk_shim_free(c->d_rr4); nntk_shim_free(c->d_rr_train); nntk_shim_free(c->d_b4); nntk_shim_free(c->d_b4_train);
     nntk_shim_free(c->d_h[0]);
     nntk_shim_host_free(c->pin_in); nntk_shim_host_free(c->pin_out); nntk_shim_host_free((void *)c->flag);
@@ -231,6 +233,7 @@
     c->wt_valid = 0;
     c->rr_valid = 0;
     c->rr_hf_valid = 0;
+    c->fk_hf_valid = 0;
     c->rr_exact_only = rr_unsplittable(c->weights->W, (size_t)c->in * G * H + (size_t)H * G * H);
     nntk_wblock_mark_uploaded(&c->wb);
     return 0;
@@ -442,6 +445,11 @@
         snprintf(buf, n, "%s: %s_rr_kernel<%d,%d> (register-resident split-bf16 x 3, input projection fused)%s; the stateful single-sequence call keeps the exact-f32 kernels",
                  cell, cell, c->H <= 256 ? 4 : 8, c->in <= 64 ? 1 : c->in <= 128 ? 2 : 4,
                  nntk_shim_lstm_rr_image_floats(c->H, c->in) != 0 ? "" : "; in % 8 != 0: the input is packed into frag3 form first");
+    if (c->G == 4 && c->return_sequences && !rr_why_not(l, c->wb.uploaded && c->rr_exact_only, nntk_shim_lstm_rr_hf_ok(c->H, c->in))) {
+        const size_t k = strlen(buf);
+        snprintf(buf + k, n - k, "; frag2h output from the zero state: lstm_rr_kernel<8,%d,hf>%s%s", c->in <= 64 ? 1 : c->in <= 128 ? 2 : 4,
+                 nntk_shim_fk_hf_ok(c->H, c->in) ? " = " : "", nntk_shim_fk_hf_ok(c->H, c->in) ? nntk_shim_fk_hf_kernel_name() : "");
+    }
     return buf;
 }
 
@@ -1671,8 +1679,16 @@
             if (nntk_shim_lstm_rr_pack_hf(c->d_ut, c->d_wp, c->d_rr_hf, c->H, c->in, us, c->hf_wscale)) return -1;
         }
         c->rr_hf_valid = 1;
+        c->fk_hf_valid = 0;
     }
     if (!(c->hf_wscale > 0.f)) return 1;
+    const int fk = nntk_shim_fk_hf_ok(c->H, c->in);
+    if (fk && !c->fk_hf_valid) {
+        size_t imgfk = nntk_shim_fk_hf_image_floats(c->H, c->in);
+        if (!c->d_fk_hf && !(c->d_fk_hf = (float *)nntk_shim_malloc(imgfk * sizeof(float)))) return -1;
+        if (nntk_shim_fk_pack_hf(c->d_ut, c->d_wp, c->d_fk_hf, c->H, c->in, c->hf_wscale / 32768.f, c->hf_wscale)) return -1;
+        c->fk_hf_valid = 1;
+    }
     const float *xf3 = d_in_f3;
     if (!xf3) {
         float *buf = nntk_devbuf_reserve(&c->d_xf3, nntk_shim_frag3_floats(B, c->T, c->in));
@@ -1681,7 +1697,8 @@
     }
     float *d_work = nntk_devbuf_reserve(&c->d_work_rr, nntk_shim_lstm_rr_work_floats(B, c->H));
     if (!d_work) return -1;
-    return nntk_shim_lstm_rr_hf(xf3, c->d_rr_hf, c->d_bi, l->use_bh ? c->d_bh : NULL, d_out_h2, d_work, B, c->T, c->in, c->H, 1.f / c->hf_wscale);
+    const float *imgfk = fk ? c->d_fk_hf : NULL;
+    return nntk_shim_lstm_rr_hf(xf3, c->d_rr_hf, imgfk, c->d_bi, l->use_bh ? c->d_bh : NULL, d_out_h2, d_work, B, c->T, c->in, c->H, 1.f / c->hf_wscale);
 }
 static int lstm_apply_device_h2(LSTM filter, const float *d_in, const float *d_in_f3, float *d_out_h2, int B) {
     rec_layer *l = &filter->l;
diff --git a/nntoolkitcore_amd/csrc/host/runtime.c b/nntoolkitcore_amd/csrc/host/runtime.c
--- a/nntoolkitcore_amd/csrc/host/runtime.c
+++ b/nntoolkitcore_amd/csrc/host/runtime.c
@@ -20,6 +20,7 @@
 int nntk_hip_get_option(const char *name, int *value) { nntk_shim_clear_error(); return nntk_shim_get_option(name, value); }
 int nntk_hip_device_status(void) { return nntk_shim_device_status(); }
 const char *nntk_hip_last_recurrent_kernel(void) { return nntk_shim_last_rec_kernel(); }
+const char *nntk_hip_last_recurrent_detail(void) { return nntk_shim_last_rec_detail(); }
 const char *nntk_hip_last_conv_kernel(void) { return nntk_shim_last_conv_kernel(); }
 
 int nntk_dist_get_unique_id(unsigned char id[NNTK_DIST_ID_BYTES]) { nntk_shim_clear_error(); return nntk_shim_dist_unique_id(id); }
```

New measurement: 73.24 million. 0.988x the previous value.
